# ljanyst/ssd-tensorflow

Measured on AMD Instinct MI355X. Metric: images/sec (fwd+bwd) vgg300 batch32, higher is better.
Workload: dtype f32; 1 GPU; vgg300 training step (forward + multibox loss + backward + momentum update), 32 images/GPU x 1 GPU, synthetic 300x300 BGR 0..255, GPU-encoded labels, Xavier-init weights (BASELINE.json configs[1]); global_batch=32, parallelism=dp1, allreduce=none

## Files before the change

### include/ssdvgg_hip.h

```cpp
#ifndef SSDVGG_HIP_H
#define SSDVGG_HIP_H

#include <stddef.h>

#ifdef __cplusplus
extern "C" {
#endif

typedef struct ssd_net* ssd_handle;

const char* ssd_last_error(void);
const char* ssd_version(void);

int ssd_preset_info(const char* preset, int* image_w, int* image_h, int* num_anchors, int* num_maps);
int ssd_preset_map(const char* preset, int map, int* size, double* scale, int* num_types);

int ssd_anchors(const char* preset, int device, double* out);
int ssd_anchors_abs(const char* preset, int device, int* out);

int ssd_jaccard_overlap(int device, const double* box, const double* boxes, int n, double* iou_out);

int ssd_encode_labels(const char* preset, int num_classes, int device, const double* gt_boxes,
                      const int* gt_cls, const int* gt_offsets, int b, float* vec_out);
int ssd_encode_labels_dev(const char* preset, int num_classes, int device, const double* gt_boxes,
// ... 231 lines not shown

size_t ssd_arena_floats(const char* preset, int num_classes);
int ssd_create(const char* preset, int num_classes, int max_batch, int device, int training,
               unsigned long long seed, float* ext_params_dev, float* ext_grads_dev,
               float* ext_momentum_dev, ssd_handle* out);
#define SSD_DTYPE_F32 0
#define SSD_DTYPE_BF16 1
#define SSD_DTYPE_FP8 2
#define SSD_DTYPE_MXFP8 3
#define SSD_DTYPE_MXFP6 4
int ssd_create_dtype(const char* preset, int num_classes, int max_batch, int device, int training,
                     unsigned long long seed, float* ext_params_dev, float* ext_grads_dev,
                     float* ext_momentum_dev, int dtype, ssd_handle* out);
int ssd_get_dtype(ssd_handle h, int* dtype);
#define SSD_GRAPH_A_TROUS 0
#define SSD_GRAPH_FC 1
size_t ssd_arena_floats_graph(const char* preset, int num_classes, int graph);
int ssd_create_graph(const char* preset, int num_classes, int max_batch, int device, int training,
                     unsigned long long seed, float* ext_params_dev, float* ext_grads_dev,
                     float* ext_momentum_dev, int dtype, int graph, ssd_handle* out);
int ssd_graph(ssd_handle h, int* graph);
int ssd_destroy(ssd_handle h);
int ssd_set_stream(ssd_handle h, void* stream);

int ssd_num_variables(ssd_handle h);
int ssd_variable_info(ssd_handle h, int i, char* name, int name_cap, int* ndim, int shape[4]);
int ssd_load_variable(ssd_handle h, const char* name, const float* data, size_t count);
int ssd_save_variable(ssd_handle h, const char* name, float* data, size_t count);
int ssd_save_gradient(ssd_handle h, const char* name, float* data, size_t count);
int ssd_save_momentum(ssd_handle h, const char* name, float* data, size_t count);
int ssd_load_momentum(ssd_handle h, const char* name, const float* data, size_t count);

int ssd_set_optimizer(ssd_handle h, const float* lr_values, const long long* lr_boundaries,
                      int n_values, float momentum, float weight_decay);
int ssd_get_global_step(ssd_handle h, long long* step);
int ssd_set_global_step(ssd_handle h, long long step);

int ssd_train_step(ssd_handle h, const float* x, const float* y, int b, float* result_out,
                   float losses_out[4]);
int ssd_eval_step(ssd_handle h, const float* x, const float* y, int b, float* result_out,
                  float losses_out[4]);
int ssd_infer(ssd_handle h, const float* x, int b, float* result_out);

int ssd_forward_backward_dev(ssd_handle h, const float* x_dev, const float* y_dev, int b);
int ssd_apply_gradients_dev(ssd_handle h, float grad_scale);
int ssd_forward_dev(ssd_handle h, const float* x_dev, const float* y_dev, int b);
int ssd_backward_begin_dev(ssd_handle h, const float* y_dev, int b);
int ssd_backward_next_dev(ssd_handle h, size_t min_floats, int sync_main, size_t* offset, size_t* count, int* more);
int ssd_backward_ranges(ssd_handle h, size_t min_floats, size_t* offsets, size_t* counts, int cap, int* n_out);
int ssd_set_wgrad_stream(ssd_handle h, void* stream);
int ssd_set_loss_normalizer(ssd_handle h, float batch);
int ssd_null_gradients_dev(ssd_handle h);
enum { SSD_LOSS_MINING = 0, SSD_LOSS_FOCAL = 1 };
typedef struct { int kind; float focal_gamma; float focal_alpha; } ssd_loss_config;
int ssd_set_loss(ssd_handle h, const ssd_loss_config* cfg);
int ssd_get_loss(ssd_handle h, ssd_loss_config* cfg);
enum { SSD_LOC_SMOOTH_L1 = 0, SSD_LOC_GIOU = 1 };
typedef struct { int kind; float weight; } ssd_loc_loss_config;
int ssd_set_loc_loss(ssd_handle h, const ssd_loc_loss_config* cfg);
int ssd_get_loc_loss(ssd_handle h, ssd_loc_loss_config* cfg);

int ssd_grads_to_bf16(int device, const float* grads_dev, void* msg_dev, size_t count, void* stream);
int ssd_grads_from_bf16(int device, const void* msg_dev, float* grads_dev, size_t count, void* stream);
int ssd_train_step_dev(ssd_handle h, const float* x_dev, const float* y_dev, int b);
int ssd_eval_step_dev(ssd_handle h, const float* x_dev, const float* y_dev, int b);
int ssd_infer_dev(ssd_handle h, const float* x_dev, int b);
int ssd_result_dev(ssd_handle h, const float** result_dev);
int ssd_get_losses(ssd_handle h, float losses_out[4]);
int ssd_get_losses_step(ssd_handle h, int steps_back, float losses_out[4]);
int ssd_get_result(ssd_handle h, int b, float* result_out);
int ssd_set_result_dev(ssd_handle h, const float* pred_dev, int b);
int ssd_arenas(ssd_handle h, float** params_dev, float** grads_dev, float** momentum_dev,
               size_t* floats, size_t* filter_floats);
int ssd_detect_last(ssd_handle h, int b, float conf_thr, int cap, int max_out, int out_cap, int nms,
                    int* count, float* conf, int* cls, int* idx, int* box);
int ssd_detect_last_dev(ssd_handle h, int b, float conf_thr, int cap, int max_out, int out_cap, int nms,
                        int** count_dev, float** conf_dev, int** cls_dev, int** idx_dev, int** box_dev);
int ssd_detect_fetch(ssd_handle h, int which, int* count, float* conf, int* cls, int* idx, int* box);
int ssd_detect_last_all_dev(ssd_handle h, int b, float conf_thr, int nms_top_k, int keep_top_k, int out_cap,
                            int** count_dev, float** conf_dev, int** cls_dev, int** idx_dev, int** box_dev);
int ssd_detect_host(ssd_handle h, int which, const int** count, const float** conf, const int** cls, const int** idx,
                    const int** box, int* b, int* out_cap);
int ssd_set_overlap(ssd_handle h, int on);
int ssd_profile_enable(ssd_handle h, int on);
int ssd_profile_report(ssd_handle h, char* buf, size_t cap);
int ssd_activation_shape(ssd_handle h, const char* name, int* height, int* width, int* channels);
int ssd_activation(ssd_handle h, const char* name, int b, float* out, size_t count);

int ssd_op_conv2d_fwd(const float* x, const float* w, const float* bias, float* y, int b, int hi,
                      int wi, int ci, int ho, int wo, int co, int kh, int kw, int stride, int dil,
                      int pad_h, int pad_w, int relu, void* stream);
int ssd_op_conv2d_dgrad(const float* dy, const float* w, float* dx, const float* mask,
                        int accumulate, int b, int hi, int wi, int ci, int ho, int wo, int co,
                        int kh, int kw, int stride, int dil, int pad_h, int pad_w, void* stream);
size_t ssd_op_conv2d_wgrad_ws_floats(int b, int hi, int wi, int ci, int ho, int wo, int co, int kh,
                                     int kw, int stride, int dil, int pad_h, int pad_w);
int ssd_op_conv2d_wgrad(const float* x, const float* dy, float* dw, float* dbias, const float* w,
                        float weight_decay, float* ws, int b, int hi, int wi, int ci, int ho, int wo,
                        int co, int kh, int kw, int stride, int dil, int pad_h, int pad_w,
                        void* stream);
int ssd_op_cast_filter(const float* w, void* w_io_bf16, void* w_oi_bf16, int taps, int ci, int co,
                       void* stream);
int ssd_op_conv2d_fwd_bf16(const void* x, const void* w_oi, const float* bias, void* y, int y_f32,
                           int b, int hi, int wi, int ci, int ho, int wo, int co, int kh, int kw,
                           int stride, int dil, int pad_h, int pad_w, int relu, void* stream);
int ssd_op_conv2d_dgrad_bf16(const void* dy, const void* w_io, void* dx, const void* mask,
                             int accumulate, int b, int hi, int wi, int ci, int ho, int wo, int co,
                             int kh, int kw, int stride, int dil, int pad_h, int pad_w, void* stream);
size_t ssd_op_conv2d_wgrad_bf16_ws_floats(int b, int hi, int wi, int ci, int ho, int wo, int co,
                                          int kh, int kw, int stride, int dil, int pad_h, int pad_w);
int ssd_op_conv2d_wgrad_bf16(const void* x, const void* dy, float* dw, float* dbias, const float* w,
                             float weight_decay, float* ws, int b, int hi, int wi, int ci, int ho,
                             int wo, int co, int kh, int kw, int stride, int dil, int pad_h,
                             int pad_w, void* stream);
int ssd_op_conv2d_fwd_bf16_chain(const void* x, const void* w_oi, const float* bias, void* y, int y_f32,
                                 int b, int hi, int wi, int ci, int ho, int wo, int co, int kh, int kw,
                                 int stride, int dil, int pad_h, int pad_w, int relu, void* stream);
int ssd_op_conv2d_dgrad_bf16_chain(const void* dy, const void* w_io, void* dx, const void* mask,
                                   int accumulate, int b, int hi, int wi, int ci, int ho, int wo, int co,
                                   int kh, int kw, int stride, int dil, int pad_h, int pad_w, void* stream);
int ssd_op_conv2d_wgrad_bf16_direct(const void* x, const void* dy, float* dw, float* dbias, const float* w,
                                    float weight_decay, int b, int hi, int wi, int ci, int ho, int wo, int co,
                                    int kh, int kw, int stride, int dil, int pad_h, int pad_w, void* stream);
typedef struct {
    int hi, wi, ci, ho, wo, co, kh, kw, stride, dil, pad_h, pad_w;
    int dgrad, relu, accum, out_f32;
    const void* src;
    const void* wgt;
    const float* bias;
    const void* mask;
    void* dst;
} ssd_tail_stage;
#define SSD_TAIL_ZERO_BYTES 2560
#define SSD_TAIL_LDS_MAX (160 * 1024)
#define SSD_TAIL_MAX_TASKS 64
#define SSD_TF_RELU 1
#define SSD_TF_ACCUM 2
#define SSD_TF_OUT_F32 4
#define SSD_TF_LOAD_IN 8
#define SSD_TF_LOAD_OUT 16
#define SSD_TF_KTAIL 32
typedef struct {
    int flags;
    int ntask, tiles, ksplit, ngroups, gpt;
    int in_off, in_bytes;
    int out_off, out_bytes;
    int scratch_off, scratch_bytes;
    unsigned tasks[SSD_TAIL_MAX_TASKS][2];
} ssd_tail_plan_stage;
int ssd_op_tail_chain_plan(const ssd_tail_stage* stages, int nstages, ssd_tail_plan_stage* plan_out, int* lds_total_out);
int ssd_op_tail_chain_bf16(const ssd_tail_stage* stages, int nstages, int b, void* stream);
typedef struct {
    int hi, wi, ci, ho, wo, co, kh, kw, stride, dil, pad_h, pad_w;
    const void* x;
    const void* dy;
    float* dw;
    float* dbias;
    const float* w;
} ssd_wgrad_item;
int ssd_op_conv2d_wgrad_group_bf16(const ssd_wgrad_item* items, int n, float weight_decay, int b, void* stream);
int ssd_op_conv2d_first_fwd_bf16(const float* x, const float* w, const float* bias, void* y, int b, int hi,
                                 int wi, int ci, int ho, int wo, int co, int kh, int kw, int stride,
                                 int dil, int pad_h, int pad_w, int relu, void* stream);
size_t ssd_op_conv2d_first_wgrad_bf16_ws_floats(int b, int hi, int wi, int ci, int ho, int wo, int co,
                                                int kh, int kw, int stride, int dil, int pad_h, int pad_w);
int ssd_op_conv2d_first_wgrad_bf16(const float* x, const void* dy, float* dw, float* dbias, const float* w,
// ... 2 lines not shown
                                   int pad_w, void* stream);
int ssd_fp8_calibrate_dev(ssd_handle h, const float* x_dev, int b, int accumulate);
int ssd_fp8_num_scales(ssd_handle h, int* count);
int ssd_fp8_scale_name(ssd_handle h, int i, char* name, int name_cap);
int ssd_fp8_get_scales(ssd_handle h, float* scales, int count);
int ssd_fp8_set_scales(ssd_handle h, const float* scales, int count);
#define SSD_FP8_OUT_BF16 0
#define SSD_FP8_OUT_F32 1
#define SSD_FP8_OUT_E4M3 2
#define SSD_FP8_OUT_BF16_E4M3 3
int ssd_op_quantize_fp8(const void* x, int x_f32, size_t n, float scale, void* y8, void* stream);
int ssd_op_absmax_bf16(const void* x, size_t n, float* out_dev, int accumulate, void* stream);
int ssd_op_quantize_filter_fp8(const float* w, void* w8, float* s_w, int taps, int ci, int co, void* stream);
int ssd_op_conv2d_fwd_fp8(const void* x8, const void* w8, float s_in, const float* s_w, const float* bias, void* y, void* y8,
                          int out_mode, float s_out, int b, int hi, int wi, int ci, int ho, int wo, int co, int kh, int kw,
                          int stride, int dil, int pad_h, int pad_w, int relu, void* stream);
int ssd_op_conv2d_fwd_fp8_bigk(const void* x8, const void* w8, float s_in, const float* s_w, const float* bias, void* y, void* y8,
                               int out_mode, float s_out, int b, int hi, int wi, int ci, int ho, int wo, int co, int kh, int kw,
                               int stride, int dil, int pad_h, int pad_w, int relu, void* stream);
int ssd_op_maxpool_fwd_fp8(const void* x8, void* y8, int b, int hi, int wi, int c, int ho, int wo, int k, int stride,
                           int pad_h, int pad_w, void* stream);
#define SSD_FP8_OUT_MX 4
#define SSD_FP8_OUT_BF16_MX 5
int ssd_op_quantize_mxfp8(const void* x, int x_f32, size_t rows, int c, void* y8, void* yscales, void* stream);
int ssd_op_conv2d_fwd_mxfp8(const void* x8, const void* xscales, const void* w8, const float* s_w, const float* bias, void* y, void* y8,
                            void* yscales, int out_mode, int b, int hi, int wi, int ci, int ho, int wo, int co, int kh, int kw,
                            int stride, int dil, int pad_h, int pad_w, int relu, void* stream);
int ssd_op_conv2d_fwd_mxfp8_bigk(const void* x8, const void* xscales, const void* w8, const float* s_w, const float* bias,
                                 void* y, void* y8, void* yscales, int out_mode,
                                 int b, int hi, int wi, int ci, int ho, int wo, int co, int kh, int kw,
                                 int stride, int dil, int pad_h, int pad_w, int relu, void* stream);
int ssd_op_maxpool_fwd_mxfp8(const void* x8, const void* xscales, void* y8, void* yscales, int b, int hi, int wi, int c, int ho, int wo,
                             int k, int stride, int pad_h, int pad_w, void* stream);
int ssd_op_quantize_mxfp6(const void* x, int x_f32, size_t rows, int c, void* y6, void* yscales, void* stream);
int ssd_op_quantize_filter_mxfp6(const float* w, void* w6, void* wscales, int taps, int ci, int co, void* stream);
int ssd_op_conv2d_fwd_mxfp6(const void* x6, const void* xscales, const void* w6, const void* wscales, const float* bias, void* y, void* y6,
                            void* yscales, int out_mode, int b, int hi, int wi, int ci, int ho, int wo, int co, int kh, int kw,
                            int stride, int dil, int pad_h, int pad_w, int relu, void* stream);
int ssd_op_maxpool_fwd_mxfp6(const void* x6, const void* xscales, void* y6, void* yscales, int b, int hi, int wi, int c, int ho, int wo,
                             int k, int stride, int pad_h, int pad_w, void* stream);
int ssd_op_maxpool_fwd(const float* x, float* y, int b, int hi, int wi, int c, int ho, int wo, int k,
                       int stride, int pad_h, int pad_w, void* stream);
int ssd_op_maxpool_bwd(const float* x, const float* dy, float* dx, int accumulate, int relu_mask,
                       int b, int hi, int wi, int c, int ho, int wo, int k, int stride, int pad_h,
                       int pad_w, void* stream);
int ssd_op_maxpool_fwd_bf16(const void* x, void* y, int b, int hi, int wi, int c, int ho, int wo, int k,
                            int stride, int pad_h, int pad_w, void* stream);
int ssd_op_maxpool_bwd_bf16(const void* x, const void* dy, void* dx, int accumulate, int relu_mask,
                            int b, int hi, int wi, int c, int ho, int wo, int k, int stride, int pad_h,
                            int pad_w, void* stream);
int ssd_op_maxpool_arg_fwd(const void* x, void* y, void* arg, int bf16, int b, int hi, int wi, int c, void* stream);
int ssd_op_maxpool_arg_bwd(const void* x, const void* arg, const void* dy, void* dx, int accumulate, int relu_mask, int bf16,
                           int b, int hi, int wi, int c, void* stream);
int ssd_op_maxpool_rec_fwd(const void* x, void* y, void* rec, int bf16, int b, int hi, int wi, int c, void* stream);
int ssd_op_maxpool_rec_bwd(const void* rec, const void* dy, void* dx, int relu_mask, int bf16, int b, int hi, int wi, int c,
                           void* stream);
int ssd_op_conv2d_fwd_pool(const float* x, const float* w, const float* bias, float* y_pool, void* rec, int b, int hi, int wi,
                           int ci, int ho, int wo, int co, int kh, int kw, int stride, int dil, int pad_h, int pad_w, void* stream);
int ssd_op_conv2d_fwd_pool_bf16(const void* x, const void* w_oi, const float* bias, void* y_pool, void* rec, int b, int hi, int wi,
                                int ci, int ho, int wo, int co, int kh, int kw, int stride, int dil, int pad_h, int pad_w,
                                void* stream);
int ssd_op_conv2d_dgrad_unpool(const float* dy, const float* w, float* dx_unpooled, const void* rec, int uh, int uw, int b, int hi,
                               int wi, int ci, int ho, int wo, int co, int kh, int kw, int stride, int dil, int pad_h, int pad_w,
                               void* stream);
int ssd_op_conv2d_dgrad_unpool_bf16(const void* dy, const void* w_io, void* dx_unpooled, const void* rec, int uh, int uw, int b,
                                    int hi, int wi, int ci, int ho, int wo, int co, int kh, int kw, int stride, int dil, int pad_h,
                                    int pad_w, void* stream);
size_t ssd_op_conv2d_dgrad_first_wgrad_bf16_ws_floats(int b, int h, int w);
int ssd_op_conv2d_dgrad_first_wgrad_bf16(const void* dy, const void* w_io, const void* mask, const float* image, float* dw1, float* dbias1,
                                         const float* w1, float weight_decay, float* ws, int b, int h, int w, void* stream);
size_t ssd_op_conv2d_wino_bits_words(int b, int hi, int wi, int ci, int ho, int wo, int co, int kh, int kw, int stride, int dil,
                                     int pad_h, int pad_w);
size_t ssd_op_conv2d_wino_ws_floats(int b, int hi, int wi, int ci, int ho, int wo, int co, int kh, int kw, int stride, int dil,
                                    int pad_h, int pad_w);
int ssd_op_conv2d_wino_fwd(const float* x, const float* w, const float* bias, float* y, float* y_pool, void* rec, void* relu_bits, float* ws,
                           int flags, int b, int hi, int wi, int ci, int ho, int wo, int co, int kh, int kw, int stride, int dil,
                           int pad_h, int pad_w, int relu, void* stream);
int ssd_op_conv2d_wino_dgrad(const float* dy, const float* w, float* dx, const float* mask, const void* mask_bits, int accumulate,
                             const void* rec, int uh, int uw, float* ws, int flags, int b, int hi, int wi, int ci, int ho, int wo, int co,
                             int kh, int kw, int stride, int dil, int pad_h, int pad_w, void* stream);
int ssd_op_conv2d_wino_wgrad(const float* x, const float* dy, float* dw, float* dbias, const float* w, float weight_decay, float* ws,
                             int flags, int b, int hi, int wi, int ci, int ho, int wo, int co, int kh, int kw, int stride, int dil,
                             int pad_h, int pad_w, void* stream);
int ssd_pool_fusion(ssd_handle h, int* out, int cap, int* count);
int ssd_debug_set_ablate(const char* tokens);

int ssd_op_clock_monitor(unsigned* out_dev, int nsamples, unsigned period_ticks, void* stream);
int ssd_op_l2norm_fwd(const float* x, const float* scale, float* y, int npix, int c, void* stream);
size_t ssd_op_l2norm_bwd_ws_floats(int npix, int c);
int ssd_op_l2norm_bwd(const float* x, const float* scale, const float* dy, float* dx, float* dscale,
                      float* ws, int npix, int c, void* stream);
int ssd_op_l2norm_fwd_bf16(const void* x, const float* scale, void* y, int npix, int c, void* stream);
int ssd_op_l2norm_bwd_bf16(const void* x, const float* scale, const void* dy, void* dx, float* dscale,
                           float* ws, int npix, int c, void* stream);

size_t ssd_op_multibox_loss_ws_bytes(int nmaps, const int* hw, const int* nj, int b_total, size_t* offsets, int* num_anchors);
int ssd_op_multibox_loss(int nmaps, const int* hw, const int* nj, int num_classes, void* const* heads, const float* labels,
                         float* result, void* ws, int b, int b_off, int b_total, float bnorm, const float* filters,
                         size_t nfilters, float weight_decay, void* stream);
int ssd_op_multibox_loss_grad(int nmaps, const int* hw, const int* nj, int num_classes, void* const* grads, int grads_bf16,
                              const float* labels, const float* result, void* ws, int b, int b_off, int b_total, void* stream);
int ssd_op_multibox_loss_ex(int nmaps, const int* hw, const int* nj, int num_classes, void* const* heads, const float* labels,
                            float* result, void* ws, int b, int b_off, int b_total, float bnorm, const float* filters,
                            size_t nfilters, float weight_decay, const ssd_loss_config* cfg, void* stream);
int ssd_op_multibox_loss_grad_ex(int nmaps, const int* hw, const int* nj, int num_classes, void* const* grads, int grads_bf16,
                                 const float* labels, const float* result, void* ws, int b, int b_off, int b_total,
                                 const ssd_loss_config* cfg, void* stream);
int ssd_op_multibox_loss_ex2(int nmaps, const int* hw, const int* nj, int num_classes, void* const* heads, const float* labels,
                             float* result, void* ws, int b, int b_off, int b_total, float bnorm, const float* filters,
                             size_t nfilters, float weight_decay, const ssd_loss_config* cfg, const ssd_loc_loss_config* loc,
                             void* stream);
int ssd_op_multibox_loss_grad_ex2(int nmaps, const int* hw, const int* nj, int num_classes, void* const* grads, int grads_bf16,
                                  const float* labels, const float* result, void* ws, int b, int b_off, int b_total,
                                  const ssd_loss_config* cfg, const ssd_loc_loss_config* loc, void* stream);

#ifdef __cplusplus
}
#endif
#endif
```

### ssd_tensorflow_amd/_lib.py

```python
import ctypes as C
import os

_HERE = os.path.dirname(os.path.abspath(__file__))
LIB_PATH = os.environ.get('SSD_LIB') or os.path.join(_HERE, 'libssdvgg_hip.so')

if not os.path.exists(LIB_PATH):
    raise ImportError(
        f'{LIB_PATH} is missing: build it with `python -c "import __graft_entry__ as g; g.build()"` '
        f'or `make -C {os.path.join(_HERE, "csrc")}` (hipcc, gfx950). There is no CPU fallback.')

try:
    import torch
except ImportError:
    torch = None

lib = C.CDLL(LIB_PATH)

p_f32 = C.POINTER(C.c_float)
p_f64 = C.POINTER(C.c_double)
p_i32 = C.POINTER(C.c_int)
p_i64 = C.POINTER(C.c_longlong)
vp = C.c_void_p
i32 = C.c_int
f32 = C.c_float
# ... 71 lines not shown
    'ssd_annotate_style_destroy': (i32, [vp]),
    'ssd_annotate_ws_bytes': (sz, [i32, i32]),
    'ssd_annotate_batch_dev': (i32, [vp, i32, vp, i32, vp, vp, vp, i32, i32, vp, i32, vp, i32, vp, vp]),
    'ssd_jpeg_info': (i32, [vp, sz, p_i32, p_i32, p_i32, p_i32, p_i32]),
    'ssd_jpeg_coef_bytes': (sz, [vp, sz]),
    'ssd_jpeg_entropy_decode': (i32, [vp, sz, vp, sz, vp, p_i32]),
    'ssd_jpeg_entropy_decode_batch': (i32, [vp, vp, i32, i32, vp, vp, vp, vp]),
    'ssd_jpeg_ws_bytes': (sz, [vp, i32]),
    'ssd_jpeg_decode_batch_dev': (i32, [vp, sz, vp, i32, vp, sz, vp, sz, vp]),
    'ssd_jpeg_scan_segments': (sz, [vp, sz]),
    'ssd_jpeg_scan_plan': (i32, [vp, sz, vp, vp, p_i32]),
    'ssd_jpeg_huffdec_ws_bytes': (sz, [vp, vp, i32]),
    'ssd_jpeg_huffdec_batch_dev': (i32, [vp, sz, vp, vp, i32, vp, sz, vp, vp, sz, i32, vp]),
    'ssd_jpeg_quant_tables': (i32, [i32, vp, vp]),
    'ssd_jpeg_enc_coef_bytes': (sz, [vp, i32, i32]),
    'ssd_jpeg_enc_ws_bytes': (sz, [vp, i32, i32]),
    'ssd_jpeg_encode_batch_dev': (i32, [vp, sz, vp, vp, i32, i32, i32, vp, sz, vp, vp, sz, vp]),
    'ssd_jpeg_file_bound': (sz, [vp]),
    'ssd_jpeg_entropy_encode': (i32, [vp, sz, vp, vp, sz, C.POINTER(sz)]),
    'ssd_jpeg_entropy_encode_batch': (i32, [vp, sz, vp, i32, i32, vp, sz, vp, vp]),
    'ssd_jpeg_file_header': (i32, [vp, vp]),
    'ssd_jpeg_huff_ws_bytes': (sz, [vp, i32]),
    'ssd_jpeg_huff_out_bytes': (sz, [vp, i32]),
    'ssd_jpeg_huffman_batch_dev': (i32, [vp, sz, vp, i32, vp, sz, vp, vp, sz, vp]),
    'ssd_sampler_trials': (i32, [vp, i32, vp, vp, i32, i32, vp, i32, vp, vp]),
    'ssd_create': (i32, [cstr, i32, i32, i32, i32, C.c_ulonglong, vp, vp, vp, C.POINTER(handle)]),
    'ssd_create_dtype': (i32, [cstr, i32, i32, i32, i32, C.c_ulonglong, vp, vp, vp, i32, C.POINTER(handle)]),
    'ssd_get_dtype': (i32, [handle, p_i32]),
    'ssd_arena_floats_graph': (sz, [cstr, i32, i32]),
    'ssd_create_graph': (i32, [cstr, i32, i32, i32, i32, C.c_ulonglong, vp, vp, vp, i32, i32, C.POINTER(handle)]),
    'ssd_graph': (i32, [handle, p_i32]),
    'ssd_destroy': (i32, [handle]),
    'ssd_set_stream': (i32, [handle, vp]),
    'ssd_num_variables': (i32, [handle]),
    'ssd_variable_info': (i32, [handle, i32, C.c_char_p, i32, p_i32, p_i32]),
    'ssd_load_variable': (i32, [handle, cstr, vp, sz]),
    'ssd_save_variable': (i32, [handle, cstr, vp, sz]),
    'ssd_save_gradient': (i32, [handle, cstr, vp, sz]),
    'ssd_save_momentum': (i32, [handle, cstr, vp, sz]),
    'ssd_load_momentum': (i32, [handle, cstr, vp, sz]),
    'ssd_set_optimizer': (i32, [handle, vp, vp, i32, f32, f32]),
    'ssd_get_global_step': (i32, [handle, p_i64]),
    'ssd_set_global_step': (i32, [handle, C.c_longlong]),
    'ssd_train_step': (i32, [handle, vp, vp, i32, vp, vp]),
    'ssd_eval_step': (i32, [handle, vp, vp, i32, vp, vp]),
    'ssd_infer': (i32, [handle, vp, i32, vp]),
    'ssd_forward_backward_dev': (i32, [handle, vp, vp, i32]),
    'ssd_apply_gradients_dev': (i32, [handle, f32]),
    'ssd_forward_dev': (i32, [handle, vp, vp, i32]),
    'ssd_backward_begin_dev': (i32, [handle, vp, i32]),
    'ssd_backward_next_dev': (i32, [handle, sz, i32, C.POINTER(sz), C.POINTER(sz), p_i32]),
    'ssd_backward_ranges': (i32, [handle, sz, C.POINTER(sz), C.POINTER(sz), i32, p_i32]),
    'ssd_set_wgrad_stream': (i32, [handle, vp]),
    'ssd_set_loss_normalizer': (i32, [handle, f32]),
    'ssd_null_gradients_dev': (i32, [handle]),
    'ssd_set_loss': (i32, [handle, vp]),
    'ssd_get_loss': (i32, [handle, vp]),
    'ssd_set_loc_loss': (i32, [handle, vp]),
    'ssd_get_loc_loss': (i32, [handle, vp]),
    'ssd_train_step_dev': (i32, [handle, vp, vp, i32]),
    'ssd_eval_step_dev': (i32, [handle, vp, vp, i32]),
    'ssd_infer_dev': (i32, [handle, vp, i32]),
    'ssd_result_dev': (i32, [handle, C.POINTER(vp)]),
    'ssd_get_result': (i32, [handle, i32, vp]),
    'ssd_get_losses': (i32, [handle, vp]),
    'ssd_get_losses_step': (i32, [handle, i32, vp]),
    'ssd_set_result_dev': (i32, [handle, vp, i32]),
    'ssd_arenas': (i32, [handle, C.POINTER(vp), C.POINTER(vp), C.POINTER(vp), C.POINTER(sz), C.POINTER(sz)]),
    'ssd_detect_last': (i32, [handle, i32, f32, i32, i32, i32, i32, vp, vp, vp, vp, vp]),
    'ssd_detect_last_dev': (i32, [handle, i32, f32, i32, i32, i32, i32, C.POINTER(vp), C.POINTER(vp), C.POINTER(vp), C.POINTER(vp), C.POINTER(vp)]),
    'ssd_detect_last_all_dev': (i32, [handle, i32, f32, i32, i32, i32, C.POINTER(vp), C.POINTER(vp), C.POINTER(vp), C.POINTER(vp), C.POINTER(vp)]),
    'ssd_detect_fetch': (i32, [handle, i32, vp, vp, vp, vp, vp]),
    'ssd_detect_host': (i32, [handle, i32, C.POINTER(vp), C.POINTER(vp), C.POINTER(vp), C.POINTER(vp), C.POINTER(vp), p_i32, p_i32]),
    'ssd_nms_boxes': (i32, [i32, i32, vp, vp, vp, C.c_double, vp, p_i32]),
    'ssd_merge_tiles_limits': (i32, [p_i32, p_i32, p_i32]),
    'ssd_merge_tiles_ws_bytes': (sz, [i32, i32]),
    'ssd_merge_tiles_dev': (i32, [vp, i32, i32, i32, vp, vp, vp, vp, vp, i32, i32, i32, vp, vp, vp, vp, vp, vp, vp, vp]),
    'ssd_merge_tiles': (i32, [i32, vp, i32, i32, i32, vp, vp, vp, vp, vp, i32, i32, i32, vp, vp, vp, vp, vp, vp]),
    'ssd_detout_tiles_ws_bytes': (sz, [cstr, i32, i32, i32, i32]),
    'ssd_detout_tiles_add_dev': (i32, [cstr, i32, vp, vp, vp, i32, i32, i32, f32, i32, i32, vp, sz, vp]),
    'ssd_detout_tiles_merge_dev': (i32, [i32, vp, i32, i32, i32, i32, i32, vp, vp, vp, vp, vp, vp, vp, sz, vp]),
    'ssd_detout_tiles': (i32, [cstr, i32, i32, vp, vp, i32, i32, f32, i32, i32, i32, i32, vp, vp, vp, vp, vp, vp]),
    'ssd_set_overlap': (i32, [handle, i32]),
    'ssd_profile_enable': (i32, [handle, i32]),
    'ssd_profile_report': (i32, [handle, C.c_char_p, sz]),
    'ssd_activation_shape': (i32, [handle, cstr, p_i32, p_i32, p_i32]),
    'ssd_activation': (i32, [handle, cstr, i32, vp, sz]),
    'ssd_op_conv2d_fwd': (i32, [vp, vp, vp, vp] + [i32] * 14 + [vp]),
    'ssd_op_conv2d_dgrad': (i32, [vp, vp, vp, vp, i32] + [i32] * 13 + [vp]),
    'ssd_op_conv2d_wgrad_ws_floats': (sz, [i32] * 13),
    'ssd_op_conv2d_wgrad': (i32, [vp, vp, vp, vp, vp, f32, vp] + [i32] * 13 + [vp]),
    'ssd_op_conv2d_wino_ws_floats': (sz, [i32] * 13),
    'ssd_op_conv2d_wino_bits_words': (sz, [i32] * 13),
    'ssd_op_conv2d_wino_fwd': (i32, [vp, vp, vp, vp, vp, vp, vp, vp, i32] + [i32] * 14 + [vp]),
    'ssd_op_conv2d_wino_dgrad': (i32, [vp, vp, vp, vp, vp, i32, vp, i32, i32, vp, i32] + [i32] * 13 + [vp]),
    'ssd_op_conv2d_wino_wgrad': (i32, [vp, vp, vp, vp, vp, f32, vp, i32] + [i32] * 13 + [vp]),
    'ssd_op_cast_filter': (i32, [vp, vp, vp, i32, i32, i32, vp]),
    'ssd_op_conv2d_fwd_bf16': (i32, [vp, vp, vp, vp, i32] + [i32] * 14 + [vp]),
    'ssd_op_conv2d_dgrad_bf16': (i32, [vp, vp, vp, vp, i32] + [i32] * 13 + [vp]),
    'ssd_op_conv2d_fwd_bf16_chain': (i32, [vp, vp, vp, vp, i32] + [i32] * 14 + [vp]),
    'ssd_op_conv2d_dgrad_bf16_chain': (i32, [vp, vp, vp, vp, i32] + [i32] * 13 + [vp]),
    'ssd_op_conv2d_wgrad_bf16_direct': (i32, [vp, vp, vp, vp, vp, f32] + [i32] * 13 + [vp]),
    'ssd_op_tail_chain_plan': (i32, [C.POINTER(TailStage), i32, C.POINTER(TailPlanStage), p_i32]),
    'ssd_op_tail_chain_bf16': (i32, [C.POINTER(TailStage), i32, i32, vp]),
    'ssd_op_conv2d_wgrad_group_bf16': (i32, [C.POINTER(WgradItem), i32, f32, i32, vp]),
    'ssd_op_conv2d_wgrad_bf16_ws_floats': (sz, [i32] * 13),
    'ssd_op_conv2d_wgrad_bf16': (i32, [vp, vp, vp, vp, vp, f32, vp] + [i32] * 13 + [vp]),
    'ssd_op_conv2d_first_fwd_bf16': (i32, [vp, vp, vp, vp] + [i32] * 14 + [vp]),
    'ssd_op_conv2d_first_wgrad_bf16_ws_floats': (sz, [i32] * 13),
    'ssd_op_conv2d_first_wgrad_bf16': (i32, [vp, vp, vp, vp, vp, f32, vp] + [i32] * 13 + [vp]),
    'ssd_op_maxpool_rec_fwd': (i32, [vp, vp, vp, i32, i32, i32, i32, i32, vp]),
    'ssd_op_maxpool_rec_bwd': (i32, [vp, vp, vp, i32, i32, i32, i32, i32, i32, vp]),
    'ssd_op_conv2d_fwd_pool': (i32, [vp, vp, vp, vp, vp] + [i32] * 13 + [vp]),
    'ssd_op_conv2d_fwd_pool_bf16': (i32, [vp, vp, vp, vp, vp] + [i32] * 13 + [vp]),
    'ssd_op_conv2d_dgrad_unpool': (i32, [vp, vp, vp, vp, i32, i32] + [i32] * 13 + [vp]),
    'ssd_op_conv2d_dgrad_unpool_bf16': (i32, [vp, vp, vp, vp, i32, i32] + [i32] * 13 + [vp]),
    'ssd_op_conv2d_dgrad_first_wgrad_bf16_ws_floats': (sz, [i32, i32, i32]),
    'ssd_op_conv2d_dgrad_first_wgrad_bf16': (i32, [vp, vp, vp, vp, vp, vp, vp, f32, vp, i32, i32, i32, vp]),
    'ssd_pool_fusion': (i32, [handle, p_i32, i32, p_i32]),
    'ssd_debug_set_ablate': (i32, [cstr]),
    'ssd_fp8_calibrate_dev': (i32, [handle, vp, i32, i32]),
    'ssd_fp8_num_scales': (i32, [handle, p_i32]),
    'ssd_fp8_scale_name': (i32, [handle, i32, C.c_char_p, i32]),
    'ssd_fp8_get_scales': (i32, [handle, vp, i32]),
    'ssd_fp8_set_scales': (i32, [handle, vp, i32]),
    'ssd_op_quantize_fp8': (i32, [vp, i32, sz, f32, vp, vp]),
    'ssd_op_absmax_bf16': (i32, [vp, sz, vp, i32, vp]),
    'ssd_op_quantize_filter_fp8': (i32, [vp, vp, vp, i32, i32, i32, vp]),
    'ssd_op_conv2d_fwd_fp8': (i32, [vp, vp, f32, vp, vp, vp, vp, i32, f32] + [i32] * 14 + [vp]),
    'ssd_op_conv2d_fwd_fp8_bigk': (i32, [vp, vp, f32, vp, vp, vp, vp, i32, f32] + [i32] * 14 + [vp]),
    'ssd_op_maxpool_fwd_fp8': (i32, [vp, vp] + [i32] * 10 + [vp]),
    'ssd_op_quantize_mxfp8': (i32, [vp, i32, sz, i32, vp, vp, vp]),
    'ssd_op_conv2d_fwd_mxfp8': (i32, [vp, vp, vp, vp, vp, vp, vp, vp, i32] + [i32] * 14 + [vp]),
    'ssd_op_conv2d_fwd_mxfp8_bigk': (i32, [vp, vp, vp, vp, vp, vp, vp, vp, i32] + [i32] * 14 + [vp]),
    'ssd_op_maxpool_fwd_mxfp8': (i32, [vp, vp, vp, vp] + [i32] * 10 + [vp]),
    'ssd_op_quantize_mxfp6': (i32, [vp, i32, sz, i32, vp, vp, vp]),
    'ssd_op_quantize_filter_mxfp6': (i32, [vp, vp, vp, i32, i32, i32, vp]),
    'ssd_op_conv2d_fwd_mxfp6': (i32, [vp, vp, vp, vp, vp, vp, vp, vp, i32] + [i32] * 14 + [vp]),
    'ssd_op_maxpool_fwd_mxfp6': (i32, [vp, vp, vp, vp] + [i32] * 10 + [vp]),
    'ssd_op_maxpool_fwd': (i32, [vp, vp] + [i32] * 10 + [vp]),
    'ssd_op_maxpool_bwd': (i32, [vp, vp, vp, i32, i32] + [i32] * 10 + [vp]),
    'ssd_op_maxpool_fwd_bf16': (i32, [vp, vp] + [i32] * 10 + [vp]),
    'ssd_op_maxpool_bwd_bf16': (i32, [vp, vp, vp, i32, i32] + [i32] * 10 + [vp]),
    'ssd_op_maxpool_arg_fwd': (i32, [vp, vp, vp, i32, i32, i32, i32, i32, vp]),
    'ssd_op_maxpool_arg_bwd': (i32, [vp, vp, vp, vp, i32, i32, i32, i32, i32, i32, i32, vp]),
    'ssd_op_clock_monitor': (i32, [vp, i32, C.c_uint, vp]),
    'ssd_grads_to_bf16': (i32, [i32, vp, vp, sz, vp]),
    'ssd_grads_from_bf16': (i32, [i32, vp, vp, sz, vp]),
    'ssd_op_l2norm_fwd': (i32, [vp, vp, vp, i32, i32, vp]),
    'ssd_op_l2norm_bwd_ws_floats': (sz, [i32, i32]),
    'ssd_op_l2norm_bwd': (i32, [vp, vp, vp, vp, vp, vp, i32, i32, vp]),
    'ssd_op_l2norm_fwd_bf16': (i32, [vp, vp, vp, i32, i32, vp]),
    'ssd_op_l2norm_bwd_bf16': (i32, [vp, vp, vp, vp, vp, vp, i32, i32, vp]),
    'ssd_op_multibox_loss_ws_bytes': (sz, [i32, p_i32, p_i32, i32, C.POINTER(sz), p_i32]),
    'ssd_op_multibox_loss': (i32, [i32, p_i32, p_i32, i32, C.POINTER(vp), vp, vp, vp, i32, i32, i32, f32, vp, sz, f32, vp]),
    'ssd_op_multibox_loss_grad': (i32, [i32, p_i32, p_i32, i32, C.POINTER(vp), i32, vp, vp, vp, i32, i32, i32, vp]),
    'ssd_op_multibox_loss_ex': (i32, [i32, p_i32, p_i32, i32, C.POINTER(vp), vp, vp, vp, i32, i32, i32, f32, vp, sz, f32, vp, vp]),
    'ssd_op_multibox_loss_grad_ex': (i32, [i32, p_i32, p_i32, i32, C.POINTER(vp), i32, vp, vp, vp, i32, i32, i32, vp, vp]),
    'ssd_op_multibox_loss_ex2': (i32, [i32, p_i32, p_i32, i32, C.POINTER(vp), vp, vp, vp, i32, i32, i32, f32, vp, sz, f32, vp, vp, vp]),
    'ssd_op_multibox_loss_grad_ex2': (i32, [i32, p_i32, p_i32, i32, C.POINTER(vp), i32, vp, vp, vp, i32, i32, i32, vp, vp, vp]),
}

for _name, (_res, _args) in SIGNATURES.items():
    _fn = getattr(lib, _name)
    _fn.restype = _res
    _fn.argtypes = _args


_device = 0


def set_device(device):
    global _device
    _device = int(device)


def device():
    return _device

# ... 17 lines not shown
```

### ssd_tensorflow_amd/csrc/api.hip

```cpp
#include "../../include/ssdvgg_hip.h"
#include "net.h"
#include "augment.h"
#include "annotate.h"
#include "jpeg.h"
#include "jpeg_enc.h"
#include "jpeg_huff.h"
#include "jpeg_huffdec.h"
#include "metrics.h"
#include <vector>
#include <map>
#include <memory>
#include <mutex>
#include <algorithm>

namespace ssd {
static thread_local std::string g_err;
void set_error(const char* fmt, ...) {
    char buf[1024];
    va_list ap;
    va_start(ap, fmt);
    vsnprintf(buf, sizeof buf, fmt, ap);
    va_end(ap);
    g_err = buf;
}
// ... 1283 lines not shown
    n.forward(n.x_stage(), b, true, n.y_stage());
    n.backward_apply(b, n.y_stage(), 1.f);
    if (result_out) n.copy_result(result_out, b);
    if (losses_out) n.get_losses(losses_out);
    HIP_OK(hipStreamSynchronize(n.stream()));
    API_END
}
int ssd_eval_step(ssd_handle h, const float* x, const float* y, int b, float* result_out, float losses_out[4]) {
    API_BEGIN_NET(h)
    n.upload_xy(x, y, b);
    n.forward(n.x_stage(), b, true, n.y_stage());
    if (result_out) n.copy_result(result_out, b);
    if (losses_out) n.get_losses(losses_out);
    HIP_OK(hipStreamSynchronize(n.stream()));
    API_END
}
int ssd_infer(ssd_handle h, const float* x, int b, float* result_out) {
    API_BEGIN_NET(h)
    n.upload_xy(x, nullptr, b);
    n.forward(n.x_stage(), b, false, nullptr);
    if (result_out) n.copy_result(result_out, b);
    HIP_OK(hipStreamSynchronize(n.stream()));
    API_END
}

int ssd_detect_last(ssd_handle h, int b, float conf_thr, int cap, int max_out, int out_cap, int nms, int* count, float* conf,
                    int* cls, int* idx, int* box) {
    API_BEGIN_NET(h)
    n.detect_last(b, conf_thr, cap, max_out, out_cap, nms != 0, count, conf, cls, idx, box);
    API_END
}

int ssd_detect_last_dev(ssd_handle h, int b, float conf_thr, int cap, int max_out, int out_cap, int nms, int** count_dev,
                        float** conf_dev, int** cls_dev, int** idx_dev, int** box_dev) {
    API_BEGIN_NET(h)
    DetectOut d{};
    n.detect_last_dev(b, conf_thr, cap, max_out, out_cap, nms != 0, &d);
    if (count_dev) *count_dev = d.count;
    if (conf_dev) *conf_dev = d.conf;
    if (cls_dev) *cls_dev = d.cls;
    if (idx_dev) *idx_dev = d.idx;
    if (box_dev) *box_dev = d.box;
    API_END
}

int ssd_detect_last_all_dev(ssd_handle h, int b, float conf_thr, int nms_top_k, int keep_top_k, int out_cap, int** count_dev,
                            float** conf_dev, int** cls_dev, int** idx_dev, int** box_dev) {
    API_BEGIN_NET(h)
    DetectOut d{};
    n.detect_last_all_dev(b, conf_thr, nms_top_k, keep_top_k, out_cap, &d);
    if (count_dev) *count_dev = d.count;
    if (conf_dev) *conf_dev = d.conf;
    if (cls_dev) *cls_dev = d.cls;
    if (idx_dev) *idx_dev = d.idx;
    if (box_dev) *box_dev = d.box;
    API_END
}

int ssd_detect_fetch(ssd_handle h, int which, int* count, float* conf, int* cls, int* idx, int* box) {
    API_BEGIN_NET(h)
    n.detect_fetch(which, count, conf, cls, idx, box);
    API_END
}

int ssd_detect_host(ssd_handle h, int which, const int** count, const float** conf, const int** cls, const int** idx,
                    const int** box, int* b, int* out_cap) {
    API_BEGIN_NET(h)
    DetectOut d;
    n.detect_host(which, &d, b, out_cap);
    if (count) *count = d.count;
    if (conf) *conf = d.conf;
    if (cls) *cls = d.cls;
    if (idx) *idx = d.idx;
    if (box) *box = d.box;
    API_END
}

int ssd_set_overlap(ssd_handle h, int on) {
    API_BEGIN_NET(h)
    n.set_overlap(on != 0);
    API_END
}

int ssd_profile_enable(ssd_handle h, int on) {
    API_BEGIN_NET(h)
    n.profiler().on = on != 0;
    n.profiler().detailed = on == 2;
    n.profiler().reset();
    API_END
}

int ssd_profile_report(ssd_handle h, char* buf, size_t cap) {
    API_BEGIN_NET(h)
    HIP_OK(hipStreamSynchronize(n.stream()));
    struct Agg { long long cnt = 0; double ms = 0, fl = 0, by = 0; };
    std::map<std::string, Agg> agg;
    for (const auto& r : n.profiler().recs) {
        float ms = 0.f;
        HIP_OK(hipEventElapsedTime(&ms, r.e0, r.e1));
        Agg& a = agg[r.kernel];
        a.cnt++; a.ms += ms; a.fl += r.flops; a.by += r.bytes;
    }
    std::string out;
    char line[384];
    for (const auto& kv : agg) {
        snprintf(line, sizeof line, "%s\t%lld\t%.6f\t%.6e\t%.6e\n", kv.first.c_str(), kv.second.cnt, kv.second.ms, kv.second.fl,
                 kv.second.by);
        out += line;
    }
    SSD_REQUIRE(buf && cap > out.size(), "report needs %zu bytes", out.size() + 1);
    memcpy(buf, out.c_str(), out.size() + 1);
    n.profiler().reset();
    API_END
}

int ssd_activation_shape(ssd_handle h, const char* name, int* height, int* width, int* channels) {
    API_BEGIN_NET(h)
    n.activation_shape(name, height, width, channels);
    API_END
}

int ssd_activation(ssd_handle h, const char* name, int b, float* out, size_t count) {
    API_BEGIN_NET(h)
    n.activation(name, b, out, count);
    API_END
}

static ConvDesc mk(int b, int hi, int wi, int ci, int ho, int wo, int co, int kh, int kw, int stride, int dil, int pad_h,
                   int pad_w) {
    ConvDesc d;
    d.B = b; d.Hi = hi; d.Wi = wi; d.Ci = ci; d.Ho = ho; d.Wo = wo; d.Co = co;
    d.KH = kh; d.KW = kw; d.stride = stride; d.dil = dil; d.pad_h = pad_h; d.pad_w = pad_w;
    return d;
}

int ssd_op_conv2d_fwd(const float* x, const float* w, const float* bias, float* y, int b, int hi, int wi, int ci, int ho,
                      int wo, int co, int kh, int kw, int stride, int dil, int pad_h, int pad_w, int relu, void* stream) {
    API_BEGIN
    conv_fwd(mk(b, hi, wi, ci, ho, wo, co, kh, kw, stride, dil, pad_h, pad_w), x, w, bias, y, relu != 0, (hipStream_t)stream);
    API_END
}
int ssd_op_conv2d_dgrad(const float* dy, const float* w, float* dx, const float* mask, int accumulate, int b, int hi, int wi,
                        int ci, int ho, int wo, int co, int kh, int kw, int stride, int dil, int pad_h, int pad_w,
                        void* stream) {
    API_BEGIN
    conv_dgrad(mk(b, hi, wi, ci, ho, wo, co, kh, kw, stride, dil, pad_h, pad_w), dy, w, dx, mask, accumulate != 0,
               (hipStream_t)stream);
    API_END
}
int ssd_op_cast_filter(const float* w, void* w_io_bf16, void* w_oi_bf16, int taps, int ci, int co, void* stream) {
    API_BEGIN
    FilterCastPlan plan;
    plan.add(0, taps, ci, co);
    cast_filters(plan, w, (bf16_t*)w_io_bf16, (bf16_t*)w_oi_bf16, (hipStream_t)stream);
    API_END
}
int ssd_op_conv2d_fwd_bf16(const void* x, const void* w_oi, const float* bias, void* y, int y_f32, int b, int hi, int wi, int ci,
                           int ho, int wo, int co, int kh, int kw, int stride, int dil, int pad_h, int pad_w, int relu,
                           void* stream) {
    API_BEGIN
    conv_fwd_bf16(mk(b, hi, wi, ci, ho, wo, co, kh, kw, stride, dil, pad_h, pad_w), (const bf16_t*)x, (const bf16_t*)w_oi, bias, y,
                  y_f32 != 0, relu != 0, (hipStream_t)stream);
    API_END
}
int ssd_op_conv2d_dgrad_bf16(const void* dy, const void* w_io, void* dx, const void* mask, int accumulate, int b, int hi, int wi,
                             int ci, int ho, int wo, int co, int kh, int kw, int stride, int dil, int pad_h, int pad_w,
// ... 133 lines not shown
    API_BEGIN
    conv_first_fwd_bf16(mk(b, hi, wi, ci, ho, wo, co, kh, kw, stride, dil, pad_h, pad_w), x, w, bias, (bf16_t*)y, relu != 0,
                        (hipStream_t)stream);
    API_END
}
size_t ssd_op_conv2d_first_wgrad_bf16_ws_floats(int b, int hi, int wi, int ci, int ho, int wo, int co, int kh, int kw, int stride,
                                                int dil, int pad_h, int pad_w) {
    return conv_first_wgrad_bf16_ws_floats(mk(b, hi, wi, ci, ho, wo, co, kh, kw, stride, dil, pad_h, pad_w));
}
int ssd_op_conv2d_first_wgrad_bf16(const float* x, const void* dy, float* dw, float* dbias, const float* w, float weight_decay,
                                   float* ws, int b, int hi, int wi, int ci, int ho, int wo, int co, int kh, int kw, int stride,
                                   int dil, int pad_h, int pad_w, void* stream) {
    API_BEGIN
    conv_first_wgrad_bf16(mk(b, hi, wi, ci, ho, wo, co, kh, kw, stride, dil, pad_h, pad_w), x, (const bf16_t*)dy, dw, dbias, w,
                          weight_decay, ws, (hipStream_t)stream);
    API_END
}
namespace {
struct WinoWs {
    float *U, *Uf, *V, *Mx, *Yt, *Ya, *slabs;
    size_t total;
    WinoWs(const ConvDesc& d, float* ws) {
        const size_t cop = wino_kpad(d.Co), u = (size_t)36 * d.Ci * cop, t = (size_t)36 * wino_tiles(d);
        U = ws; Uf = U + u; V = Uf + u; Mx = V + t * d.Ci; Yt = Mx + t * std::max((size_t)d.Ci, cop); Ya = Yt + t * cop; slabs = Ya + t * cop;
        total = (size_t)(slabs - ws) + wino_wgrad_ws_floats(d);
    }
};
}
size_t ssd_op_conv2d_wino_ws_floats(int b, int hi, int wi, int ci, int ho, int wo, int co, int kh, int kw, int stride, int dil,
                                    int pad_h, int pad_w) {
    const ConvDesc d = mk(b, hi, wi, ci, ho, wo, co, kh, kw, stride, dil, pad_h, pad_w);
    return wino_applicable(d) ? WinoWs(d, nullptr).total : 0;
}
size_t ssd_op_conv2d_wino_bits_words(int b, int hi, int wi, int ci, int ho, int wo, int co, int kh, int kw, int stride, int dil,
                                     int pad_h, int pad_w) {
    const ConvDesc d = mk(b, hi, wi, ci, ho, wo, co, kh, kw, stride, dil, pad_h, pad_w);
    return wino_applicable(d) ? (size_t)wino_tiles(d) * (d.Ci / 4) : 0;
}
int ssd_op_conv2d_wino_fwd(const float* x, const float* w, const float* bias, float* y, float* y_pool, void* rec, void* relu_bits, float* ws,
                           int flags, int b, int hi, int wi, int ci, int ho, int wo, int co, int kh, int kw, int stride, int dil,
                           int pad_h, int pad_w, int relu, void* stream) {
    API_BEGIN
    const ConvDesc d = mk(b, hi, wi, ci, ho, wo, co, kh, kw, stride, dil, pad_h, pad_w);
    SSD_REQUIRE(wino_applicable(d), "winograd: 3x3 / stride 1 / SAME layers (any dilation), Ci in multiples of 32, Co of 4");
    const WinoWs k(d, ws);
    if (!(flags & 1)) {
        HIP_OK(hipMemsetAsync(k.Uf, 0, (size_t)36 * d.Ci * wino_kpad(d.Co) * sizeof(float), (hipStream_t)stream));
        wino_filter(d, w, k.U, k.Uf, (hipStream_t)stream);
    }
    wino_fwd(d, x, k.U, bias, y, relu != 0, k.V, (size_t)wino_tiles(d) * d.Ci, k.Mx, y_pool, rec, (hipStream_t)stream, relu_bits,
             (flags & 4) != 0, (flags & 8) != 0);
    API_END
}
int ssd_op_conv2d_wino_dgrad(const float* dy, const float* w, float* dx, const float* mask, const void* mask_bits, int accumulate,
                             const void* rec, int uh, int uw, float* ws, int flags, int b, int hi, int wi, int ci, int ho, int wo, int co,
                             int kh, int kw, int stride, int dil, int pad_h, int pad_w, void* stream) {
    API_BEGIN
    const ConvDesc d = mk(b, hi, wi, ci, ho, wo, co, kh, kw, stride, dil, pad_h, pad_w);
    SSD_REQUIRE(wino_applicable(d), "winograd: 3x3 / stride 1 / SAME layers (any dilation), Ci in multiples of 32, Co of 4");
    const WinoWs k(d, ws);
    if (!(flags & 1)) {
        HIP_OK(hipMemsetAsync(k.Uf, 0, (size_t)36 * d.Ci * wino_kpad(d.Co) * sizeof(float), (hipStream_t)stream));
        wino_filter(d, w, k.U, k.Uf, (hipStream_t)stream);
    }
    wino_bwd_transform(d, dy, k.Yt, nullptr, (hipStream_t)stream, (flags & 8) != 0);
    wino_dgrad(d, k.Yt, k.Uf, dx, mask, accumulate != 0, k.Mx, rec, uh, uw, (hipStream_t)stream, mask_bits, (flags & 4) != 0);
    API_END
}
int ssd_op_conv2d_wino_wgrad(const float* x, const float* dy, float* dw, float* dbias, const float* w, float weight_decay, float* ws,
                             int flags, int b, int hi, int wi, int ci, int ho, int wo, int co, int kh, int kw, int stride, int dil,
                             int pad_h, int pad_w, void* stream) {
    API_BEGIN
    const ConvDesc d = mk(b, hi, wi, ci, ho, wo, co, kh, kw, stride, dil, pad_h, pad_w);
    SSD_REQUIRE(wino_applicable(d), "winograd: 3x3 / stride 1 / SAME layers (any dilation), Ci in multiples of 32, Co of 4");
    const WinoWs k(d, ws);
    const size_t vps = (size_t)wino_tiles(d) * d.Ci;
    if (!(flags & 2)) {
        ConvDesc dx = d;
        dx.Co = d.Ci; dx.Ho = d.Hi; dx.Wo = d.Wi;
        wino_bwd_transform(dx, x, k.V, nullptr, (hipStream_t)stream, (flags & 8) != 0);
    }
    wino_bwd_transform(d, dy, nullptr, k.Ya, (hipStream_t)stream, (flags & 8) != 0);
    wino_wgrad(d, k.V, vps, k.Ya, dw, dbias, w, weight_decay, k.slabs, (hipStream_t)stream, (flags & 8) != 0);
    API_END
}
size_t ssd_op_conv2d_wgrad_ws_floats(int b, int hi, int wi, int ci, int ho, int wo, int co, int kh, int kw, int stride,
                                     int dil, int pad_h, int pad_w) {
    return conv_wgrad_ws_floats(mk(b, hi, wi, ci, ho, wo, co, kh, kw, stride, dil, pad_h, pad_w));
}
int ssd_op_conv2d_wgrad(const float* x, const float* dy, float* dw, float* dbias, const float* w, float weight_decay,
                        float* ws, int b, int hi, int wi, int ci, int ho, int wo, int co, int kh, int kw, int stride, int dil,
                        int pad_h, int pad_w, void* stream) {
    API_BEGIN
    conv_wgrad(mk(b, hi, wi, ci, ho, wo, co, kh, kw, stride, dil, pad_h, pad_w), x, dy, dw, dbias, w, weight_decay, ws,
               (hipStream_t)stream);
    API_END
}
int ssd_op_quantize_fp8(const void* x, int x_f32, size_t n, float scale, void* y8, void* stream) {
    API_BEGIN
    quantize_fp8(x, x_f32 != 0, n, scale, (unsigned char*)y8, (hipStream_t)stream);
    API_END
}
int ssd_op_absmax_bf16(const void* x, size_t n, float* out_dev, int accumulate, void* stream) {
    API_BEGIN
    absmax_bf16((const bf16_t*)x, n, out_dev, accumulate != 0, (hipStream_t)stream);
    API_END
}
int ssd_op_quantize_filter_fp8(const float* w, void* w8, float* s_w, int taps, int ci, int co, void* stream) {
    API_BEGIN
    SSD_REQUIRE(w && w8 && s_w && taps >= 1 && ci >= 1 && co >= 1, "quantize_filter_fp8: null argument or empty filter");
    FilterQuantPlan plan;
    plan.add(0, 0, 0, taps, ci, co);
    quantize_filters_fp8(plan, w, (unsigned char*)w8, s_w, (hipStream_t)stream);
    API_END
}
int ssd_op_conv2d_fwd_fp8(const void* x8, const void* w8, float s_in, const float* s_w, const float* bias, void* y, void* y8,
                          int out_mode, float s_out, int b, int hi, int wi, int ci, int ho, int wo, int co, int kh, int kw, int stride,
                          int dil, int pad_h, int pad_w, int relu, void* stream) {
    API_BEGIN
    conv_fwd_fp8(mk(b, hi, wi, ci, ho, wo, co, kh, kw, stride, dil, pad_h, pad_w), (const unsigned char*)x8, (const unsigned char*)w8, s_in,
                 s_w, bias, y, (unsigned char*)y8, out_mode, s_out, relu != 0, (hipStream_t)stream);
    API_END
}
int ssd_op_conv2d_fwd_fp8_bigk(const void* x8, const void* w8, float s_in, const float* s_w, const float* bias, void* y, void* y8,
                               int out_mode, float s_out, int b, int hi, int wi, int ci, int ho, int wo, int co, int kh, int kw, int stride,
                               int dil, int pad_h, int pad_w, int relu, void* stream) {
    API_BEGIN
    conv_bigk_fwd_fp8(mk(b, hi, wi, ci, ho, wo, co, kh, kw, stride, dil, pad_h, pad_w), (const unsigned char*)x8, (const unsigned char*)w8,
                      s_in, s_w, bias, y, (unsigned char*)y8, out_mode, s_out, relu != 0, (hipStream_t)stream);
    API_END
}
int ssd_op_maxpool_fwd_fp8(const void* x8, void* y8, int b, int hi, int wi, int c, int ho, int wo, int k, int stride, int pad_h,
                           int pad_w, void* stream) {
    API_BEGIN
    PoolDesc d{b, hi, wi, c, ho, wo, k, stride, pad_h, pad_w};
    maxpool_fwd_fp8(d, (const unsigned char*)x8, (unsigned char*)y8, (hipStream_t)stream);
    API_END
}
int ssd_op_quantize_mxfp8(const void* x, int x_f32, size_t rows, int c, void* y8, void* yscales, void* stream) {
    API_BEGIN
    quantize_mxfp8(x, x_f32 != 0, rows, c, (unsigned char*)y8, (unsigned char*)yscales, (hipStream_t)stream);
    API_END
}
int ssd_op_conv2d_fwd_mxfp8(const void* x8, const void* xscales, const void* w8, const float* s_w, const float* bias, void* y, void* y8,
                            void* yscales, int out_mode, int b, int hi, int wi, int ci, int ho, int wo, int co, int kh, int kw, int stride,
                            int dil, int pad_h, int pad_w, int relu, void* stream) {
    API_BEGIN
    conv_fwd_mxfp8(mk(b, hi, wi, ci, ho, wo, co, kh, kw, stride, dil, pad_h, pad_w), (const unsigned char*)x8, (const unsigned char*)xscales,
                   (const unsigned char*)w8, s_w, bias, y, (unsigned char*)y8, (unsigned char*)yscales, out_mode, relu != 0, (hipStream_t)stream);
    API_END
}
int ssd_op_conv2d_fwd_mxfp8_bigk(const void* x8, const void* xscales, const void* w8, const float* s_w, const float* bias, void* y, void* y8,
                                 void* yscales, int out_mode, int b, int hi, int wi, int ci, int ho, int wo, int co, int kh, int kw, int stride,
                                 int dil, int pad_h, int pad_w, int relu, void* stream) {
    API_BEGIN
    conv_bigk_fwd_mxfp8(mk(b, hi, wi, ci, ho, wo, co, kh, kw, stride, dil, pad_h, pad_w), (const unsigned char*)x8, (const unsigned char*)xscales,
                        (const unsigned char*)w8, s_w, bias, y, (unsigned char*)y8, (unsigned char*)yscales, out_mode, relu != 0, (hipStream_t)stream);
    API_END
}
int ssd_op_maxpool_fwd_mxfp8(const void* x8, const void* xscales, void* y8, void* yscales, int b, int hi, int wi, int c, int ho, int wo, int k,
                             int stride, int pad_h, int pad_w, void* stream) {
    API_BEGIN
    PoolDesc d{b, hi, wi, c, ho, wo, k, stride, pad_h, pad_w};
    maxpool_fwd_mxfp8(d, (const unsigned char*)x8, (const unsigned char*)xscales, (unsigned char*)y8, (unsigned char*)yscales, (hipStream_t)stream);
    API_END
}
// ... 334 lines not shown
```

### ssd_tensorflow_amd/csrc/conv.h

```cpp
#pragma once
#include <vector>
#include "common.h"

namespace ssd {

struct ConvDesc {
    int B, Hi, Wi, Ci;
    int Ho, Wo, Co;
    int KH, KW, stride, dil;
    int pad_h, pad_w;
};

void conv_fwd(const ConvDesc& d, const float* x, const float* w, const float* bias,
              float* y, bool relu, hipStream_t s);

void conv_dgrad(const ConvDesc& d, const float* dy, const float* w, float* dx,
                const float* mask, bool accumulate, hipStream_t s);

size_t conv_wgrad_ws_floats(const ConvDesc& d);
void conv_wgrad(const ConvDesc& d, const float* x, const float* dy, float* dw, float* dbias,
                const float* w, float weight_decay, float* ws, hipStream_t s);

bool conv_fwd_pool_supported(const ConvDesc& d);
void conv_fwd_pool(const ConvDesc& d, const float* x, const float* w, const float* bias, float* y_pool, void* rec, hipStream_t s);
bool conv_dgrad_unpool_supported(const ConvDesc& d);
void conv_dgrad_unpool(const ConvDesc& d, const float* dy, const float* w, float* dx_unpooled, const void* rec, int UH, int UW,
                       hipStream_t s);

bool conv_first_fwd_f32_applicable(const ConvDesc& d);
void conv_first_fwd_f32(const ConvDesc& d, const float* x, const float* w, const float* bias, float* y, bool relu, hipStream_t s);
bool conv_first_wgrad_f32_applicable(const ConvDesc& d);
size_t conv_first_wgrad_f32_ws_floats(const ConvDesc& d);
void conv_first_wgrad_f32(const ConvDesc& d, const float* x, const float* dy, float* dw, float* dbias, const float* w,
                          float weight_decay, float* ws, hipStream_t s);

bool wino_applicable(const ConvDesc& d);
int wino_tiles(const ConvDesc& d);
int wino_kpad(int c);
void wino_filter(const ConvDesc& d, const float* w, float* U, float* Uflip, hipStream_t s);
struct WinoFilterPlan {
    static constexpr int MAX = 24;
    struct Item {
        const float* w;
        float *U, *Uf;
        int Ci, Co, Cop, blk0;
    } it[MAX];
    int n = 0, blocks = 0;
    double elems = 0;
    void add(const float* w, float* U, float* Uf, int Ci, int Co);
};
void wino_filter_plan(const WinoFilterPlan& plan, bool forward, bool flipped, hipStream_t s);
size_t wino_fwd_ws_floats(const ConvDesc& d);
void wino_fwd(const ConvDesc& d, const float* x, const float* U, const float* bias, float* y, bool relu, float* V, size_t v_ps,
              float* Mws, float* y_pool, void* pool_rec, hipStream_t s, void* relu_bits = nullptr, bool two_launch = false,
              bool ref_geom = false);
void wino_bwd_transform(const ConvDesc& d, const float* dy, float* Yt, float* Ya, hipStream_t s, bool ref_geom = false);
size_t wino_dgrad_ws_floats(const ConvDesc& d);
void wino_dgrad(const ConvDesc& d, const float* Yt, const float* Uflip, float* dx, const float* mask, bool accumulate, float* Xws,
                const void* unpool_rec, int UH, int UW, hipStream_t s, const void* mask_bits = nullptr, bool two_launch = false);
size_t wino_wgrad_ws_floats(const ConvDesc& d);
void wino_wgrad(const ConvDesc& d, const float* V, size_t v_ps, const float* Ya, float* dw, float* dbias, const float* w,
                float weight_decay, float* ws, hipStream_t s, bool ref_geom = false);

bool conv_bigk(const ConvDesc& d);
double conv_bigk_useful_flops(const ConvDesc& d);
void conv_bigk_fwd(const ConvDesc& d, const float* x, const float* w, const float* bias, float* y, bool relu, hipStream_t s);
void conv_bigk_dgrad(const ConvDesc& d, const float* dy, const float* w, float* dx, const float* mask, bool accumulate, hipStream_t s);
void conv_bigk_wgrad(const ConvDesc& d, const float* x, const float* dy, float* dw, float* dbias, const float* w, float weight_decay,
                     hipStream_t s);

struct bf16_t;

void conv_fwd_smallc_bf16out(const ConvDesc& d, const float* x, const float* w, const float* bias, bf16_t* y, bool relu,
                             hipStream_t s);
void conv_wgrad_smallc_bf16dy(const ConvDesc& d, const float* x, const bf16_t* dy, float* dw, float* dbias, const float* w,
                              float weight_decay, float* ws, hipStream_t s);

void conv_first_fwd_bf16(const ConvDesc& d, const float* x, const float* w, const float* bias, bf16_t* y, bool relu, hipStream_t s);
size_t conv_first_wgrad_bf16_ws_floats(const ConvDesc& d);
void conv_first_wgrad_bf16(const ConvDesc& d, const float* x, const bf16_t* dy, float* dw, float* dbias, const float* w,
                           float weight_decay, float* ws, hipStream_t s);

void conv_bigk_fwd_bf16(const ConvDesc& d, const bf16_t* x, const bf16_t* w_oi, const float* bias, void* y, bool y_f32, bool relu,
                        hipStream_t s);
void conv_bigk_dgrad_bf16(const ConvDesc& d, const bf16_t* dy, const bf16_t* w_io, bf16_t* dx, const bf16_t* mask, bool accumulate,
                          hipStream_t s);
void conv_bigk_wgrad_bf16(const ConvDesc& d, const bf16_t* x, const bf16_t* dy, float* dw, float* dbias, const float* w,
                          float weight_decay, hipStream_t s);

struct FilterCastPlan {
    static constexpr int MAX_LAYERS = 48;
    struct Layer {
        size_t off;
        int taps, ci, co;
    } L[MAX_LAYERS];
    int n = 0;
    void add(size_t off, int taps, int ci, int co);
};
void cast_filters(const FilterCastPlan& plan, const float* w, bf16_t* io, bf16_t* oi, hipStream_t s);

extern thread_local int g_conv_lanes;
void conv_fwd_bf16(const ConvDesc& d, const bf16_t* x, const bf16_t* w_oi, const float* bias, void* y, bool y_f32, bool relu,
                   hipStream_t s);
void conv_dgrad_bf16(const ConvDesc& d, const bf16_t* dy, const bf16_t* w_io, bf16_t* dx, const bf16_t* mask, bool accumulate,
                     hipStream_t s);
bool conv_fwd_pool_bf16_supported(const ConvDesc& d);
void conv_fwd_pool_bf16(const ConvDesc& d, const bf16_t* x, const bf16_t* w_oi, const float* bias, bf16_t* y_pool, void* rec, hipStream_t s);
bool conv_dgrad_unpool_bf16_supported(const ConvDesc& d);
void conv_dgrad_unpool_bf16(const ConvDesc& d, const bf16_t* dy, const bf16_t* w_io, bf16_t* dx_unpooled, const void* rec, int UH, int UW,
                            hipStream_t s);
bool conv_dgrad_first_wgrad_bf16_applicable(const ConvDesc& d, const ConvDesc& d1);
size_t conv_dgrad_first_wgrad_bf16_ws_floats(const ConvDesc& d1);
void conv_dgrad_first_wgrad_bf16(const ConvDesc& d, const bf16_t* dy, const bf16_t* w_io, const bf16_t* mask, const ConvDesc& d1,
                                 const float* image, float* dw1, float* dbias1, const float* w1, float weight_decay, float* ws,
                                 hipStream_t s);
size_t conv_wgrad_bf16_ws_floats(const ConvDesc& d);
void conv_wgrad_bf16(const ConvDesc& d, const bf16_t* x, const bf16_t* dy, float* dw, float* dbias, const float* w,
                     float weight_decay, float* ws, hipStream_t s);

struct TailStage {
    ConvDesc d;
    bool dgrad;
    const void* src;
    const void* wgt_packed;
    const float* bias;
    const void* mask;
    void* dst;
    bool relu, accum, out_f32;
};
int tail_chain_max_stages();
bool tail_chain_stage_supported(const ConvDesc& d);
size_t tail_chain_packed_elems(const ConvDesc& d, bool dgrad);
struct TailPackItem {
    ConvDesc d;
    bool dgrad;
    const void* mirror;
    void* packed;
};
void tail_chain_pack_filters(const TailPackItem* items, int n, hipStream_t s);
// ... 72 lines not shown
```

### ssd_tensorflow_amd/csrc/net.h

```cpp
#pragma once
#include "common.h"
#include "conv.h"
#include "ops.h"
#include "boxes.h"
#include "bf16.h"
#include "quant_layout.h"
#include <string>
#include <vector>
#include <map>

namespace ssd {

struct Tensor {
    std::string name;
    int H = 0, W = 0, C = 0;
    bool relu_out = false;
    int consumers = 0;
    int done = 0;
    int gstream = 0;
    long gseq = 0;
    hipEvent_t gev = nullptr;
    bool gev_set = false;
    bool data_f32 = true;
    bool grad_f32 = true;
// ... 42 lines not shown
    size_t off, rows, width, pitch;
    size_t count() const { return rows * width; }
};

struct DetectSlot {
    char* dev = nullptr;
    char* host = nullptr;
    size_t bytes = 0, used = 0;
    int b = 0, out_cap = 0;
    hipEvent_t ready = nullptr;
};

class Net {
public:
    Net(const char* preset, int num_classes, int max_batch, int device, bool training, unsigned long long seed,
        float* ext_params, float* ext_grads, float* ext_momentum, int dtype = 0, int graph = 0);
    ~Net();

    static size_t arena_floats(const char* preset, int num_classes, int graph = 0);

    void set_stream(hipStream_t s) { stream_ = s; }
    hipStream_t stream() const { return stream_; }

    void forward(const float* x, int b, bool train_mode, const float* y);
    void backward(int b, const float* y);
    void backward_begin(int b, const float* y);
    bool backward_step(size_t min_floats, size_t* off, size_t* count, bool sync_main);
    std::vector<std::pair<size_t, size_t>> backward_ranges(size_t min_floats) const;
    void set_wgrad_stream(hipStream_t s);
    void apply_gradients(float grad_scale);
    void backward_apply(int b, const float* y, float grad_scale);
    void set_loss_normalizer(float bnorm) { loss_bnorm_ = bnorm; }
    void set_loss(int kind, float gamma, float alpha) { loss_kind_ = kind; focal_gamma_ = gamma; focal_alpha_ = alpha; }
    void get_loss(int* kind, float* gamma, float* alpha) const { *kind = loss_kind_; *gamma = focal_gamma_; *alpha = focal_alpha_; }
    void set_loc_loss(int kind, float weight) { loc_.kind = kind; loc_.weight = weight; }
    void get_loc_loss(int* kind, float* weight) const { *kind = loc_.kind; *weight = loc_.weight; }
    void null_gradients_step();
    void set_optimizer(const float* lr_values, const long long* bounds, int n, float momentum, float wd);

    void upload_xy(const float* x, const float* y, int b);
    const float* x_stage() const { return x_stage_; }
    const float* y_stage() const { return y_stage_; }

    void get_losses(float out[4]);
    void get_losses_step(int steps_back, float out[4]);
    void copy_result(float* out, int b);
    void set_result(const float* pred_dev, int b);

    const std::vector<Variable>& variables() const { return vars_; }
    void load_variable(const char* name, const float* host, size_t count, int which);
    void save_variable(const char* name, float* host, size_t count, int which);
    void activation(const char* name, int b, float* out, size_t count);
    void activation_shape(const char* name, int* H, int* W, int* C) const;
    void pool_fusion(int* out, int cap, int* count) const;

    void detect_last(int b, float thr, int cap, int max_out, int out_cap, bool nms, int* count, float* conf, int* cls, int* idx, int* box);
    const DetectSlot& detect_last_dev(int b, float thr, int cap, int max_out, int out_cap, bool nms, DetectOut* dev_out);
    const DetectSlot& detect_last_all_dev(int b, float thr, int nms_top_k, int keep_top_k, int out_cap, DetectOut* dev_out);
    void detect_fetch(int which, int* count, float* conf, int* cls, int* idx, int* box);
    void detect_host(int which, DetectOut* host, int* b, int* out_cap);

    const Preset& preset() const { return *preset_; }
    int num_classes() const { return C_; }
    int nvars() const { return C_ + 5; }
    int max_batch() const { return Bmax_; }
    bool training() const { return training_; }
    int dtype() const { return quant_ == Quant::fp8 ? 2 : quant_ == Quant::mxfp8 ? 3 : quant_ == Quant::mxfp6 ? 4 : bf16_ ? 1 : 0; }
    void fp8_calibrate(const float* x_dev, int b, bool accumulate);
    int fp8_num_scales() const;
    const char* fp8_scale_name(int i) const;
    void fp8_get_scales(float* out, int n) const;
    void fp8_set_scales(const float* v, int n);
    int graph() const { return fc_ ? 1 : 0; }
    int device() const { return device_; }
    float* params() { return params_; }
    float* grads() { return grads_; }
    float* momentum() { return mom_; }
    size_t nparams() const { return nparams_; }
    size_t nfilters() const { return nfilters_; }
    float* result() { return result_; }
    long long global_step = 0;
    Profiler& profiler() { return prof_; }
    void set_overlap(bool on) { overlap_ = on; }

private:
    int add_tensor(const std::string& name, int H, int W, int C, bool relu_out);
    void build_graph();
    void alloc();
    void init_weights(unsigned long long seed);
    ConvDesc conv_desc(const Op& op, int b) const;
    float current_lr() const;
    const Variable& find_var(const char* name) const;

    const Preset* preset_;
    int C_, Bmax_, device_;
    bool training_;
    bool bf16_ = false;
    bool fc_ = false;
    Quant quant_ = Quant::none;
    unsigned char* wsc6_ = nullptr;
    QView q_at(const Tensor& t, int b0) const;
    bool fp8_calibrated_ = false, fp8_as_bf16_ = false;
    unsigned char* w8_ = nullptr;
    float *sw8_ = nullptr, *absmax8_ = nullptr;
    FilterQuantPlan quant_plan_;
    std::vector<int> fp8_scaled_;
    void plan_fp8();
    void fp8_share_pool_scales();
    void require_fp8() const;
    bf16_t *wq_io_ = nullptr, *wq_oi_ = nullptr;
    FilterCastPlan cast_plan_;
    hipStream_t stream_ = nullptr;
    hipStream_t wstream_ = nullptr;
    hipEvent_t ev_dy_ = nullptr, ev_w_ = nullptr;
    hipStream_t hstream_ = nullptr;
    hipEvent_t ev_h_ = nullptr, ev_cast_ = nullptr, ev_fmap_[MAX_MAPS] = {};
    hipStream_t s2_ = nullptr;
    hipEvent_t ev2_h_ = nullptr, ev_l2_ = nullptr, ev_join_ = nullptr, ev2_fmap_[MAX_MAPS] = {};
    int tail_first_ = 0;
    std::vector<int> fwd_order_, bwd_order_;
    struct BwProgress {
        const Net* net = nullptr;
        std::vector<char> done;
        bool chain_done = false;
        int pos = 0;
        size_t hi = 0, lo = 0;
        void begin(const Net* n);
        int next(size_t min_floats);
        bool finished() const;
        size_t retire(int op_index);
        void retire_chain();
        std::pair<size_t, size_t> end_stage();
    private:
        size_t final_lo() const;
    } bw_;
    long bw_issued_[2] = {0, 0}, bw_seen_[2][2] = {{0, 0}, {0, 0}};
    hipEvent_t ev_m2s_ = nullptr;
    bool bw_first_on_main_ = false;
    bool fuse_first_wgrad_ = false;
    bool bw_first_fused_ = false;
    int fused_first_out_ = -1;
    void launch_wgrad(int op_index, int b, hipStream_t ws);
    void launch_dgrad(const Op& op, const ConvDesc& d, const Op* up, Tensor& dst, bool mask, int cls, hipStream_t ds);
    int chain_first_ = -1;
    std::vector<char> in_chain_;
    bf16_t* wq_tail_ = nullptr;
    std::vector<long long> tail_fwd_off_, tail_bwd_off_;
    void pack_tail_filters(hipStream_t s);
    bool chain_fwd_ = false, chain_bwd_ = false;
    void plan_tail_chain();
    void plan_winograd();
    long long fwd_serial_ = 0;
    WinoFilterPlan wino_plan_, wino_plan_first_, wino_plan_flip_;
    bool wino_flip_pending_ = false;
    bool wino_any_f_ = false, wino_any_d_ = false;
    float *wino_m_[3] = {nullptr, nullptr, nullptr}, *wino_vs_[3] = {nullptr, nullptr, nullptr}, *wino_yt_ = nullptr, *wino_xw_ = nullptr, *wino_ya_ = nullptr, *wino_slab_ = nullptr;
    hipEvent_t ev_wino_ = nullptr, ev_wino_first_ = nullptr, ev_wino_flip_ = nullptr;
    struct Lane {
        hipStream_t s, h;
        hipEvent_t* ev_fmap;
        hipEvent_t ev_h;
        int b0, nb;
        bool heads_on_side, cast_pending;
        int wino_pending;
        bool fmap_carried[MAX_MAPS];
    };
    struct FwdPass {
        Lane lane[2];
        int nl, nl_cur;
        bool heads_full;
        int small_heads;
        int b;
        bool train_mode, run8, side;
    };
    struct LossSlotGuard;
    struct ConvRun;
    void forward_filters(FwdPass& p, LossSlotGuard& guard);
    void forward_conv(FwdPass& p, int li, int op_index);
    bool conv_stream(FwdPass& p, int li, const Op& op, ConvRun& r);
    void conv_wino_scratch(const FwdPass& p, int li, int op_index, const ConvDesc& d, ConvRun& r);
    void launch_conv_fwd(const FwdPass& p, const Op& op, const ConvDesc& d, const ConvRun& r);
    void forward_pool(FwdPass& p, int li, int op_index);
    void forward_l2norm(FwdPass& p, int li, int op_index);
    void forward_loss(FwdPass& p, const float* y, LossSlotGuard& guard);
    void launch_tail_forward(int b0, int nb, hipStream_t s);
    void launch_tail_backward(int b, bool* side_used);
    void build_orders();
    void plan_pool_fusion();
    int bw_class(const Op& op, int op_index) const;
    void bw_sync(int x, int y);
    void bw_need(int x, const Tensor& t);
    void bw_wrote(int x, Tensor& t, bool carried = false);
    bool overlap_ = true;

    std::vector<Tensor> tensors_;
    std::vector<Op> ops_;
    std::vector<Variable> vars_;
    int input_t_ = -1;
    std::vector<int> head_t_;
    HeadLayout heads_{};

    size_t nparams_ = 0, nfilters_ = 0, scale_off_ = 0;
    float *params_ = nullptr, *grads_ = nullptr, *mom_ = nullptr;

    float* result_ = nullptr;
    float *x_stage_ = nullptr, *y_stage_ = nullptr;
    float* wgrad_ws_ = nullptr;
    float* l2_ws_ = nullptr;
    void* pool_ws_ = nullptr;
    int pool_arg_op_ = -1;
    void* loss_ws_ = nullptr;
    LossWork lw_{};
    static constexpr int LOSS_RING = 4;
    float* losses_host_ = nullptr;
    float* losses_dev_ = nullptr;
    hipEvent_t ev_loss_[LOSS_RING] = {};
    long long loss_seq_ = -1;
    float* begin_loss_slot();
    double* anchors_dev_ = nullptr;
    int* anchors_abs_dev_ = nullptr;
    void* detect_ws_ = nullptr;
    void* detout_ws_ = nullptr;
    size_t detout_ws_bytes_ = 0;
    DetectSlot& detect_slot_next(int b, int out_cap);
    DetectSlot det_slot_[2];
    int det_cur_ = 0;
    void detect_slot_carve(const DetectSlot& sl, DetectOut& d, char* base) const;

    std::vector<float> lr_values_{0.001f};
    std::vector<long long> lr_bounds_;
    float momentum_ = 0.9f, wd_ = 0.0005f;
    float loss_bnorm_ = 0.f;
    int loss_kind_ = 0;
    int bw_loss_kind_ = 0;
    float focal_gamma_ = 2.f, focal_alpha_ = 0.25f, bw_gamma_ = 2.f, bw_alpha_ = 0.25f;
    LocLoss loc_{}, bw_loc_{};
    Profiler prof_;
    int bw_b_ = 0;
    HipOwner hip_;
    TailTables tail_tables_{hip_, {}};
// ... 4 lines not shown
```

### ssd_tensorflow_amd/csrc/net.hip

```cpp
#include "net.h"
#include <cmath>
#include <algorithm>
#include <cstdlib>
#include <atomic>
#include <mutex>

namespace ssd {

static bool first_layer_kernel(const ConvDesc& d) { return d.Ci * d.KH * d.KW <= 32 && d.Co == 64; }

int Net::add_tensor(const std::string& name, int H, int W, int C, bool relu_out) {
    Tensor t;
    t.name = name; t.H = H; t.W = W; t.C = C; t.relu_out = relu_out;
    tensors_.push_back(t);
    return (int)tensors_.size() - 1;
}

enum PadMode { PAD_SAME, PAD_VALID, PAD_BR1_VALID };

void Net::build_graph() {
    const Preset& p = *preset_;
    const int nv = C_ + 5;
    input_t_ = add_tensor("image_input", p.image_h, p.image_w, 3, false);
    int cur = input_t_;
// ... 389 lines not shown
        t.wgt_packed = wq_tail_ + tail_fwd_off_[oi];
        t.bias = params_ + op.b_off;
        t.dst = static_cast<char*>(out.data) + (size_t)b0 * out.per_image() * (out.data_f32 ? 4 : 2);
        t.relu = op.relu; t.accum = false; t.out_f32 = out.data_f32;
        st.push_back(t);
    }
    prof_.layer = "tail";
    tail_chain_bf16(st.data(), (int)st.size(), nb, "tail_fwd_bf16", s, tail_tables_);
}

void Net::launch_tail_backward(int b, bool* side_used) {
    const bool side = hstream_ && overlap_;
    const int cls = side ? 1 : 0;
    hipStream_t ds = cls == 1 ? hstream_ : stream_;
    std::vector<TailStage> st;
    std::vector<Tensor*> written;
    Tensor* first_out = &tensors_[ops_[chain_first_].out];
    for (const int oi : bwd_order_) {
        if (!in_chain_[oi] || oi == chain_first_) continue;
        const Op& op = ops_[oi];
        Tensor& in = tensors_[op.in];
        const Tensor& out = tensors_[op.out];
        bw_need(cls, out);
        const bool last = in.done + 1 == in.consumers;
        TailStage t{};
        t.d = conv_desc(op, 1);
        t.dgrad = true;
        t.src = out.grad;
        t.wgt_packed = wq_tail_ + tail_bwd_off_[oi];
        t.mask = (last && in.relu_out) ? in.data : nullptr;
        t.dst = in.grad;
        t.accum = in.done > 0;
        st.push_back(t);
        in.done++;
        if (std::find(written.begin(), written.end(), &in) == written.end()) written.push_back(&in);
    }
    prof_.layer = "tail";
    const bool carry = first_out->gev != nullptr;
    g_stop_event = carry ? first_out->gev : nullptr;
    {
        struct Disarm { ~Disarm() { g_stop_event = nullptr; } } disarm;
        tail_chain_bf16(st.data(), (int)st.size(), b, "tail_dgrad_bf16", ds, tail_tables_);
    }
    for (Tensor* t : written) {
        t->gstream = cls;
        t->gseq = ++bw_issued_[cls];
        t->gev_set = false;
    }
    if (carry) first_out->gev_set = true;
    const bool wside = wstream_ && overlap_;
    hipStream_t ws = wside ? wstream_ : stream_;
    if (wside || cls == 1) {
        if (carry) {
            HIP_OK(hipStreamWaitEvent(ws, first_out->gev, 0));
        } else {
            HIP_OK(hipEventRecord(ev_dy_, ds));
            HIP_OK(hipStreamWaitEvent(ws, ev_dy_, 0));
        }
        if (!wside) bw_seen_[0][1] = bw_issued_[1];
    }
    std::vector<WgradGroupItem> items;
    for (int oi = 0; oi < (int)ops_.size(); ++oi) {
        if (!in_chain_[oi]) continue;
        const Op& op = ops_[oi];
        const Tensor& in = tensors_[op.in];
        const Tensor& out = tensors_[op.out];
        WgradGroupItem it{};
        it.d = conv_desc(op, b);
        if (oi == chain_first_) continue;
        it.x = in.h(); it.dy = out.gh();
        it.dw = grads_ + op.w_off; it.dbias = grads_ + op.b_off; it.w = params_ + op.w_off;
        items.push_back(it);
    }
    conv_wgrad_group_bf16(items.data(), (int)items.size(), wd_, ws);
    bw_.retire_chain();
    if (wside) *side_used = true;
}

void Net::plan_winograd() {
    if (bf16_) return;
    const int mode = env_i("SSD_WINOGRAD", 15), min_cc = env_i("SSD_WINO_MIN_CC", 4096), head_min_hw = env_i("SSD_WINO_HEAD_MIN_HW", 16);
    if (!(mode & 7)) return;
    size_t m_max = 0, v_max = 0, yt_max = 0, xw_max = 0, slab_max = 0;
    for (Op& op : ops_) {
        if (op.kind != OP_CONV) continue;
        const ConvDesc d = conv_desc(op, Bmax_);
        if (!wino_applicable(d) || d.Ci * d.Co < min_cc) continue;
        if (d.Ci > 1024) continue;
        if (op.head >= 0 && (d.Ho < head_min_hw || !(mode & 8))) continue;
        op.wino_f = (mode & 1) != 0;
        op.wino_d = (mode & 2) != 0 && training_ && op.in != input_t_;
        op.wino_w = (mode & 4) != 0 && training_ && op.wino_f;
        if (!(op.wino_f || op.wino_d)) continue;
        const size_t u = (size_t)36 * d.Ci * d.Co, uf = (size_t)36 * d.Ci * wino_kpad(d.Co), t = (size_t)36 * wino_tiles(d);
        if (op.wino_f) {
            op.wino_U = (float*)hip_.mem(u * sizeof(float));
            if (training_) op.wino_V = (float*)hip_.mem(t * d.Ci * sizeof(float));
            else v_max = std::max(v_max, t * d.Ci);
            m_max = std::max(m_max, t * d.Co);
        }
        if (op.wino_f && op.wino_d) op.wino_bits = hip_.mem((size_t)wino_tiles(d) * (d.Ci / 4) * 8);
        if (op.wino_d) {
            op.wino_Uf = (float*)hip_.mem(uf * sizeof(float));
            HIP_OK(hipMemset(op.wino_Uf, 0, uf * sizeof(float)));
            yt_max = std::max(yt_max, t * wino_kpad(d.Co));
            xw_max = std::max(xw_max, t * d.Ci);
        }
        if (op.wino_w) {
            yt_max = std::max(yt_max, t * wino_kpad(d.Co));
            for (int b = 1; b <= Bmax_; ++b) slab_max = std::max(slab_max, wino_wgrad_ws_floats(conv_desc(op, b)));
        }
        (wino_plan_first_.n == 0 && op.wino_f ? wino_plan_first_ : wino_plan_).add(params_ + op.w_off, op.wino_U, nullptr, d.Ci, d.Co);
        if (op.wino_Uf) wino_plan_flip_.add(params_ + op.w_off, nullptr, op.wino_Uf, d.Ci, d.Co);
        wino_any_f_ |= op.wino_f;
        wino_any_d_ |= op.wino_d;
    }
    if (wino_plan_.n + wino_plan_first_.n + wino_plan_flip_.n == 0) return;
    ev_wino_ = hip_.event();
    ev_wino_first_ = hip_.event();
    ev_wino_flip_ = hip_.event();
    if (m_max) for (int l = 0; l < 3; ++l) wino_m_[l] = (float*)hip_.mem(m_max * sizeof(float));
    if (v_max) for (int l = 0; l < 3; ++l) wino_vs_[l] = (float*)hip_.mem(v_max * sizeof(float));
    if (training_) {
        wino_yt_ = (float*)hip_.mem(yt_max * sizeof(float));
        wino_xw_ = (float*)hip_.mem(xw_max * sizeof(float));
        wino_ya_ = (float*)hip_.mem(yt_max * sizeof(float));
        wino_slab_ = (float*)hip_.mem(slab_max * sizeof(float));
    }
}

void Net::plan_fp8() {
    size_t nsw = 0;
    for (Tensor& t : tensors_) t.wants16 = false;
    std::vector<int> producer(tensors_.size(), -1);
    for (int i = 0; i < (int)ops_.size(); ++i) {
        Op& op = ops_[i];
        producer[op.out] = i;
        if (op.kind != OP_CONV) continue;
        const ConvDesc d = conv_desc(op, Bmax_);
        const bool kernel8 = !conv_bigk(d) ? conv_fwd_fp8_supported(d, nullptr) && conv_fwd_fp8_worthwhile(d) && (quant_ != Quant::mxfp6 || conv_fwd_mxfp6_supported(d, nullptr))
                             : quant_ == Quant::mxfp6 ? false
                             : quant_ == Quant::mxfp8 ? conv_bigk_fwd_mxfp8_supported(d, FP8_OUT_BF16_MX, nullptr) && conv_bigk_fwd_mxfp8_worthwhile(d)
                                                      : conv_bigk_fwd_fp8_supported(d, nullptr) && conv_bigk_fwd_fp8_worthwhile(d);
        op.fp8 = op.head < 0 && i < tail_first_ && !tensors_[op.in].data_f32 && kernel8;
    }
    auto need8 = [&](Tensor& t) {
        if (!t.data8) t.data8 = static_cast<unsigned char*>(hip_.mem(t.per_image() * Bmax_));
        if (quant_block_scales(quant_) && !t.scale8)
            t.scale8 = static_cast<unsigned char*>(hip_.mem(quant_scale_bytes(quant_, t.per_image()) * Bmax_ + 8));
    };
    for (int i = (int)ops_.size() - 1; i >= 0; --i) {
        Op& op = ops_[i];
        Tensor& in = tensors_[op.in];
        Tensor& out = tensors_[op.out];
        if (op.kind == OP_POOL) {
            const int prod = producer[op.in];
            op.fp8 = out.data8 != nullptr && prod >= 0 && ops_[prod].kind == OP_CONV && ops_[prod].fp8;
            if (op.fp8) {
                need8(in);
                if (out.wants16) in.wants16 = true;
            } else {
                in.wants16 = true;
            }
        } else if (op.kind == OP_CONV && op.fp8) {
            need8(in);
        } else {
            in.wants16 = true;
        }
    }
    for (int t : head_t_) tensors_[t].wants16 = true;
    size_t nw6 = 0;
    for (Op& op : ops_) {
        if (op.kind == OP_CONV && op.fp8 && quant_ == Quant::mxfp6) {
            const Tensor& in = tensors_[op.in];
            const Tensor& out = tensors_[op.out];
            const size_t n = (size_t)op.KH * op.KW * out.C * in.C;
            op.sw_off = nsw;
            op.w8_off = nw6;
            quant_plan_.add(op.w_off, nw6, nsw, op.KH * op.KW, in.C, out.C);
            nw6 += (quant_code_bytes(quant_, n) + 15) / 16 * 16;
            nsw += (quant_scale_bytes(quant_, n) + 15) / 16 * 16;
        } else if (op.kind == OP_CONV && op.fp8) {
            const Tensor& in = tensors_[op.in];
            const Tensor& out = tensors_[op.out];
            op.sw_off = nsw;
            op.w8_off = op.w_off;
            quant_plan_.add(op.w_off, op.w8_off, nsw, op.KH * op.KW, in.C, out.C);
            nsw += out.C;
        }
        Tensor& out = tensors_[op.out];
        if (!out.data8) continue;
        if (!op.fp8) out.wants16 = true;
        if (!(op.kind == OP_POOL && op.fp8) && quant_tensor_scale(quant_)) fp8_scaled_.push_back(op.out);
    }
    SSD_REQUIRE(quant_plan_.n > 0, "no layer of this graph is eligible for fp8");
    if (quant_ == Quant::mxfp6) {
        w8_ = static_cast<unsigned char*>(hip_.mem(nw6));
        wsc6_ = static_cast<unsigned char*>(hip_.mem(nsw + 8));
        return;
    }
    w8_ = static_cast<unsigned char*>(hip_.mem(nfilters_));
    sw8_ = static_cast<float*>(hip_.mem(nsw * sizeof(float)));
    if (quant_tensor_scale(quant_)) absmax8_ = static_cast<float*>(hip_.mem(fp8_scaled_.size() * sizeof(float)));
}

QView Net::q_at(const Tensor& t, int b0) const {
    return QView{t.data8 ? t.data8 + (size_t)b0 * quant_code_bytes(quant_, t.per_image()) : nullptr,
                 t.scale8 ? t.scale8 + (size_t)b0 * quant_scale_bytes(quant_, t.per_image()) : nullptr, t.scale};
}

// ... 144 lines not shown
                }
                op.ws_off = ws_total;
                ws_total += (ws + 63) / 64 * 64;
            }
        wgrad_ws_ = (float*)hip_.mem(ws_total * sizeof(float));
        l2_ws_ = (float*)hip_.mem(l2norm_bwd_ws_floats(B * 64 * 64, 512) * sizeof(float));
        size_t pws = 0;
        for (auto& op : ops_)
            if (op.kind == OP_POOL) {
                const Tensor& in = tensors_[op.in];
                const Tensor& out = tensors_[op.out];
                PoolDesc d{B, in.H, in.W, in.C, out.H, out.W, op.k, op.stride, op.pad_h, op.pad_w};
                pws = std::max(pws, maxpool_bwd_ws_bytes(d));
            }
        pool_ws_ = hip_.mem(pws);
        for (auto& op : ops_)
            if (op.kind == OP_POOL) {
                const Tensor& in = tensors_[op.in];
                const Tensor& out = tensors_[op.out];
                PoolDesc d{B, in.H, in.W, in.C, out.H, out.W, op.k, op.stride, op.pad_h, op.pad_w};
                if (maxpool_rec_applicable(d) && in.consumers == 1) op.pool_rec = hip_.mem(maxpool_rec_bytes(d));
            }
    }
    result_ = (float*)hip_.mem((size_t)B * A * nv * sizeof(float));
    x_stage_ = (float*)hip_.mem((size_t)B * preset_->image_h * preset_->image_w * 3 * sizeof(float));
    y_stage_ = (float*)hip_.mem((size_t)B * A * nv * sizeof(float));
    loss_ws_ = hip_.mem(loss_work_bytes(B, A));
    loss_work_carve(lw_, loss_ws_, B, A);
    HIP_OK(hipMemset(loss_ws_, 0, loss_work_bytes(B, A)));
    void* dp = nullptr;
    losses_host_ = static_cast<float*>(hip_.pinned(LOSS_RING * 4 * sizeof(float), &dp));
    for (int i = 0; i < LOSS_RING * 4; ++i) losses_host_[i] = 0.f;
    losses_dev_ = static_cast<float*>(dp);
    lw_.losses = losses_dev_;
    for (int i = 0; i < LOSS_RING; ++i) ev_loss_[i] = hip_.event();
    anchors_dev_ = (double*)hip_.mem((size_t)A * 4 * sizeof(double));
    anchors_abs_dev_ = (int*)hip_.mem((size_t)A * 4 * sizeof(int));
    anchors_device(*preset_, anchors_dev_, anchors_abs_dev_, nullptr);
    HIP_OK(hipDeviceSynchronize());
}

static inline double urand(unsigned long long& s) {
    unsigned long long z = (s += 0x9E3779B97F4A7C15ull);
    z = (z ^ (z >> 30)) * 0xBF58476D1CE4E5B9ull;
    z = (z ^ (z >> 27)) * 0x94D049BB133111EBull;
    z ^= z >> 31;
    return (double)(z >> 11) * (1.0 / 9007199254740992.0);
}

void Net::init_weights(unsigned long long seed) {
    std::vector<float> h(nparams_, 0.f);
    unsigned long long s = seed * 0x2545F4914F6CDD1Dull + 1;
    for (const Variable& v : vars_) {
        if (v.ndim == 4) {
            const double fan_in = (double)v.shape[0] * v.shape[1] * v.shape[2];
            const double fan_out = (double)v.shape[0] * v.shape[1] * v.shape[3];
            const double lim = std::sqrt(6.0 / (fan_in + fan_out));
            for (size_t r = 0; r < v.rows; ++r)
                for (size_t c = 0; c < v.width; ++c) h[v.off + r * v.pitch + c] = (float)((urand(s) * 2.0 - 1.0) * lim);
        } else if (v.name == "l2_norm_conv4_3/scale") {
            for (size_t c = 0; c < v.width; ++c) h[v.off + c] = 20.f;
        }
    }
    HIP_OK(hipMemcpy(params_, h.data(), nparams_ * sizeof(float), hipMemcpyHostToDevice));
}

Net::Net(const char* preset, int num_classes, int max_batch, int device, bool training, unsigned long long seed,
         float* ext_params, float* ext_grads, float* ext_momentum, int dtype, int graph)
    : preset_(&get_preset(preset)), C_(num_classes), Bmax_(max_batch), device_(device), training_(training), bf16_(dtype >= 1 && dtype <= 4),
      fc_(graph == 1), quant_(dtype == 2 ? Quant::fp8 : dtype == 3 ? Quant::mxfp8 : dtype == 4 ? Quant::mxfp6 : Quant::none), hip_(device) {
    SSD_REQUIRE(dtype >= 0 && dtype <= 4, "dtype must be 0 (fp32), 1 (bf16), 2 (fp8), 3 (mxfp8) or 4 (mxfp6), got %d", dtype);
    SSD_REQUIRE(!(quant_ != Quant::none && training), "%s is inference only: create the handle with training = 0",
                quant_ == Quant::mxfp6 ? "SSD_DTYPE_MXFP6" : quant_ == Quant::mxfp8 ? "SSD_DTYPE_MXFP8" : "SSD_DTYPE_FP8");
    SSD_REQUIRE(graph == 0 || graph == 1, "graph must be 0 (a-trous) or 1 (fc), got %d", graph);
    require_num_classes(num_classes);
    SSD_REQUIRE(max_batch >= 1, "max_batch must be >= 1");
    HIP_OK(hipSetDevice(device));
    params_ = ext_params; grads_ = ext_grads; mom_ = ext_momentum;
    build_graph();
    alloc();
    init_weights(seed);
    const char* ov = getenv("SSD_OVERLAP_WGRAD");
    overlap_ = !(ov && ov[0] == '0');
    hstream_ = hip_.stream();
    ev_h_ = hip_.event();
    ev_cast_ = hip_.event();

    ev2_h_ = hip_.event();
    ev_l2_ = hip_.event();
    ev_join_ = hip_.event();
    ev_m2s_ = hip_.event();
    for (int i = 0; i < MAX_MAPS; ++i) ev2_fmap_[i] = hip_.event();
    for (int i = 0; i < MAX_MAPS; ++i) ev_fmap_[i] = hip_.event();
    if (training_) {
        wstream_ = hip_.stream();
        ev_dy_ = hip_.event();
        ev_w_ = hip_.event();
    }
    s2_ = training_ ? wstream_ : hip_.stream();
    if (quant_ != Quant::none) plan_fp8();
    plan_pool_fusion();
    plan_tail_chain();
    plan_winograd();
    if (training_)
        for (const Op& op : ops_)
            if (op.in != input_t_ && !tensors_[op.in].gev)
                tensors_[op.in].gev = hip_.event();
    bw_.begin(this);
}

Net::~Net() {
    if (g_prof == &prof_) g_prof = nullptr;
}

static char* at(const Tensor& t, int b0, bool grad = false) {
    return static_cast<char*>(grad ? t.grad : t.data) + (size_t)b0 * t.per_image() * ((grad ? t.grad_f32 : t.data_f32) ? 4 : 2);
}

static void quantize_q(Quant q, const Tensor& t, const void* src, int nb, QView dst, hipStream_t s) {
    switch (q) {
    case Quant::mxfp6: quantize_mxfp6(src, false, (size_t)nb * t.H * t.W, t.C, dst.codes, dst.scales, s); break;
    case Quant::mxfp8: quantize_mxfp8(src, false, (size_t)nb * t.H * t.W, t.C, dst.codes, dst.scales, s); break;
    case Quant::fp8: quantize_fp8(src, false, (size_t)nb * t.per_image(), dst.scale, dst.codes, s); break;
    case Quant::none: fail("quantize: the handle has no quantised format");
    }
}

static void quantize_filters_q(Quant q, const FilterQuantPlan& plan, const float* w, unsigned char* w8, float* sw8, unsigned char* wsc6, hipStream_t s) {
    if (q == Quant::mxfp6) quantize_filters_mxfp6(plan, w, w8, wsc6, s);
    else quantize_filters_fp8(plan, w, w8, sw8, s);
}

static void conv_fwd_q(Quant q, const ConvDesc& d, QView x, const unsigned char* w, const float* sw, const unsigned char* wsc, const float* bias,
                       void* y, QView y8, bool wants16, bool relu, hipStream_t s) {
    const int mx_mode = y8.codes ? (wants16 ? FP8_OUT_BF16_MX : FP8_OUT_MX) : FP8_OUT_BF16;
    switch (q) {
    case Quant::mxfp6:
        conv_fwd_mxfp6(d, x.codes, x.scales, w, wsc, bias, y, y8.codes, y8.scales, mx_mode, relu, s);
        break;
    case Quant::mxfp8:
        (conv_bigk(d) ? conv_bigk_fwd_mxfp8 : conv_fwd_mxfp8)(d, x.codes, x.scales, w, sw, bias, y, y8.codes, y8.scales, mx_mode, relu, s);
        break;
    case Quant::fp8:
        (conv_bigk(d) ? conv_bigk_fwd_fp8 : conv_fwd_fp8)(d, x.codes, w, x.scale, sw, bias, y, y8.codes,
                                                          y8.codes ? (wants16 ? FP8_OUT_BF16_E4M3 : FP8_OUT_E4M3) : FP8_OUT_BF16, y8.scale, relu, s);
        break;
    case Quant::none: fail("convolution: the handle has no quantised format");
    }
}

static void maxpool_fwd_q(Quant q, const PoolDesc& d, QView x, QView y, hipStream_t s) {
    switch (q) {
    case Quant::mxfp6: maxpool_fwd_mxfp6(d, x.codes, x.scales, y.codes, y.scales, s); break;
    case Quant::mxfp8: maxpool_fwd_mxfp8(d, x.codes, x.scales, y.codes, y.scales, s); break;
    case Quant::fp8: maxpool_fwd_fp8(d, x.codes, y.codes, s); break;
    case Quant::none: fail("max-pool: the handle has no quantised format");
    }
}

struct Net::LossSlotGuard {
    long long& seq;
    bool armed = false;
    bool done = false;
    explicit LossSlotGuard(long long& s) : seq(s) {}
    void failed() { if (armed && !done) { --seq; armed = false; } }
    ~LossSlotGuard() { if (armed && !done) --seq; }
// ... 218 lines not shown
}

void Net::forward_pool(FwdPass& p, int li, int op_index) {
    const Op& op = ops_[op_index];
    const Tensor& in = tensors_[op.in];
    const Tensor& out = tensors_[op.out];
    const Lane& ln = p.lane[li];
    if (op.fused_fwd) return;
    PoolDesc d{ln.nb, in.H, in.W, in.C, out.H, out.W, op.k, op.stride, op.pad_h, op.pad_w};
    if (op.pool_rec && p.train_mode) {
        void* rec = static_cast<char*>(op.pool_rec) + (size_t)ln.b0 * out.H * out.W * (in.C / 4) * sizeof(unsigned short);
        if (bf16_) maxpool_fwd_rec(d, reinterpret_cast<const bf16_t*>(at(in, ln.b0)), reinterpret_cast<bf16_t*>(at(out, ln.b0)), rec, ln.s);
        else maxpool_fwd_rec(d, reinterpret_cast<const float*>(at(in, ln.b0)), reinterpret_cast<float*>(at(out, ln.b0)), rec, ln.s);
    } else if (p.train_mode && pool_ws_ && maxpool_arg_applicable(d)) {
        void* arg = static_cast<char*>(pool_ws_) + (size_t)ln.b0 * out.H * out.W * (in.C / 4) * sizeof(unsigned);
        if (bf16_) maxpool_fwd_arg(d, reinterpret_cast<const bf16_t*>(at(in, ln.b0)), reinterpret_cast<bf16_t*>(at(out, ln.b0)), arg, ln.s);
        else maxpool_fwd_arg(d, reinterpret_cast<const float*>(at(in, ln.b0)), reinterpret_cast<float*>(at(out, ln.b0)), arg, ln.s);
        pool_arg_op_ = op_index;
    } else if (p.run8 && op.fp8) {
        maxpool_fwd_q(quant_, d, q_at(in, ln.b0), q_at(out, ln.b0), ln.s);
        if (out.wants16) maxpool_fwd(d, reinterpret_cast<const bf16_t*>(at(in, ln.b0)), reinterpret_cast<bf16_t*>(at(out, ln.b0)), ln.s);
    } else if (bf16_) {
        maxpool_fwd(d, reinterpret_cast<const bf16_t*>(at(in, ln.b0)), reinterpret_cast<bf16_t*>(at(out, ln.b0)), ln.s);
        if (p.run8 && out.data8)
            quantize_q(quant_, out, at(out, ln.b0), ln.nb, q_at(out, ln.b0), ln.s);
    } else maxpool_fwd(d, reinterpret_cast<const float*>(at(in, ln.b0)), reinterpret_cast<float*>(at(out, ln.b0)), ln.s);
}

void Net::forward_l2norm(FwdPass& p, int li, int op_index) {
    const Op& op = ops_[op_index];
    const Tensor& in = tensors_[op.in];
    const Tensor& out = tensors_[op.out];
    const Lane& ln = p.lane[li];
    if (bf16_) l2norm_fwd(ln.nb * in.H * in.W, in.C, reinterpret_cast<const bf16_t*>(at(in, ln.b0)), params_ + scale_off_,
                          reinterpret_cast<bf16_t*>(at(out, ln.b0)), ln.s);
    else l2norm_fwd(ln.nb * in.H * in.W, in.C, reinterpret_cast<const float*>(at(in, ln.b0)), params_ + scale_off_,
                    reinterpret_cast<float*>(at(out, ln.b0)), ln.s);
}

void Net::forward_loss(FwdPass& p, const float* y, LossSlotGuard& guard) {
    const int b = p.b;
    const bool train_mode = p.train_mode;
    prof_.layer = "loss";
    const int A = preset_->num_anchors, nv = C_ + 5;
    if (train_mode) { bw_loss_kind_ = loss_kind_; bw_gamma_ = focal_gamma_; bw_alpha_ = focal_alpha_; bw_loc_ = loc_; }
    const bool focal = train_mode && bw_loss_kind_ == 1;
    try {
    if (p.heads_full) {
        HIP_OK(hipEventRecord(ev_h_, hstream_));
        HIP_OK(hipStreamWaitEvent(stream_, ev_h_, 0));
        HIP_OK(hipEventRecord(ev_join_, s2_));
        HIP_OK(hipStreamWaitEvent(stream_, ev_join_, 0));
        if (focal) multibox_focal_loss(heads_, b, 0, b, result_, y, lw_, wd_, loss_bnorm_, bw_gamma_, bw_alpha_, stream_, bw_loc_);
        else if (train_mode) multibox_loss(heads_, b, 0, b, result_, y, lw_, wd_, loss_bnorm_, stream_, bw_loc_);
        else heads_result(heads_, b, result_, stream_);
    }
    for (int li = 0; li < p.nl && !p.heads_full; ++li) {
        Lane& ln = p.lane[li];
        if (ln.heads_on_side) {
            HIP_OK(hipEventRecord(ln.ev_h, ln.h));
            HIP_OK(hipStreamWaitEvent(ln.s, ln.ev_h, 0));
        }
        HeadLayout hl = heads_;
        for (int i = 0; i < hl.nmaps; ++i) hl.buf[i] = heads_.buf[i] + (size_t)ln.b0 * hl.hw[i] * hl.ld[i];
        float* res = result_ + (size_t)ln.b0 * A * nv;
        if (train_mode) {
            if (li == 1) HIP_OK(hipStreamWaitEvent(ln.s, ev_l2_, 0));
            if (focal) multibox_focal_loss(hl, ln.nb, ln.b0, b, res, y + (size_t)ln.b0 * A * nv, lw_, wd_, loss_bnorm_, bw_gamma_, bw_alpha_, ln.s, bw_loc_);
            else multibox_loss(hl, ln.nb, ln.b0, b, res, y + (size_t)ln.b0 * A * nv, lw_, wd_, loss_bnorm_, ln.s, bw_loc_);
        } else {
            heads_result(hl, ln.nb, res, ln.s);
        }
    }
    } catch (...) {
        if (train_mode && lw_.ticket) {
            (void)hipDeviceSynchronize();
            (void)hipMemset(lw_.ticket, 0, sizeof(unsigned));
        }
        guard.failed();
        throw;
    }
}

void Net::launch_wgrad(int op_index, int b, hipStream_t ws) {
    const Op& op = ops_[op_index];
    const Tensor& in = tensors_[op.in];
    const Tensor& out = tensors_[op.out];
    const ConvDesc d = conv_desc(op, b);
    float* slab = wgrad_ws_ + op.ws_off;
    prof_.layer = op.name.c_str();
    if (op.wino_w && op.wino_v_step == fwd_serial_) {
        const size_t tpi = (size_t)wino_tiles(d) / d.B;
        wino_bwd_transform(d, out.gf(), nullptr, wino_ya_, ws);
        wino_wgrad(d, op.wino_V, (size_t)b * tpi * d.Ci, wino_ya_, grads_ + op.w_off, grads_ + op.b_off, params_ + op.w_off, wd_,
                   wino_slab_, ws);
    } else if (!bf16_) {
        conv_wgrad(d, in.f(), out.gf(), grads_ + op.w_off, grads_ + op.b_off, params_ + op.w_off, wd_, slab, ws);
    } else if (in.data_f32) {
        if (first_layer_kernel(d))
            conv_first_wgrad_bf16(d, in.f(), out.gh(), grads_ + op.w_off, grads_ + op.b_off, params_ + op.w_off, wd_, slab, ws);
        else
            conv_wgrad_smallc_bf16dy(d, in.f(), out.gh(), grads_ + op.w_off, grads_ + op.b_off, params_ + op.w_off, wd_, slab, ws);
    } else {
        conv_wgrad_bf16(d, in.h(), out.gh(), grads_ + op.w_off, grads_ + op.b_off, params_ + op.w_off, wd_, slab, ws);
    }
}

void Net::launch_dgrad(const Op& op, const ConvDesc& d, const Op* up, Tensor& dst, bool mask, int cls, hipStream_t ds) {
    const Tensor& in = tensors_[op.in];
    const Tensor& out = tensors_[op.out];
    if (op.wino_d && cls == 0) {
        wino_bwd_transform(d, out.gf(), wino_yt_, nullptr, ds);
        wino_dgrad(d, wino_yt_, op.wino_Uf, up ? dst.gf() : in.gf(), mask ? in.f() : nullptr, !up && in.done > 0, wino_xw_,
                   up ? up->pool_rec : nullptr, dst.H, dst.W, ds,
                   op.wino_bits && op.wino_bits_step == fwd_serial_ ? op.wino_bits : nullptr);
    } else if (!bf16_) {
        if (up) conv_dgrad_unpool(d, out.gf(), params_ + op.w_off, dst.gf(), up->pool_rec, dst.H, dst.W, ds);
        else conv_dgrad(d, out.gf(), params_ + op.w_off, in.gf(), mask ? in.f() : nullptr, in.done > 0, ds);
    } else {
        if (up) conv_dgrad_unpool_bf16(d, out.gh(), wq_io_ + op.w_off, dst.gh(), up->pool_rec, dst.H, dst.W, ds);
        else conv_dgrad_bf16(d, out.gh(), wq_io_ + op.w_off, in.gh(), mask ? in.h() : nullptr, in.done > 0, ds);
    }
}

void Net::backward_begin(int b, const float* y) {
    SSD_REQUIRE(training_, "handle was created with training = 0");
    g_prof = &prof_;
    prof_.layer = "loss";
    const bool side = hstream_ && overlap_;
    for (Tensor& t : tensors_) { t.done = 0; t.gstream = 0; t.gseq = 0; t.gev_set = false; }
    bw_issued_[0] = bw_issued_[1] = 0;
    bw_seen_[0][0] = bw_seen_[0][1] = bw_seen_[1][0] = bw_seen_[1][1] = 0;
    if (wino_flip_pending_) {
        HIP_OK(hipStreamWaitEvent(stream_, ev_wino_flip_, 0));
        wino_flip_pending_ = false;
    }
    if (bw_loss_kind_ == 1) multibox_focal_loss_grad(heads_, b, 0, result_, y, lw_, bw_gamma_, bw_alpha_, stream_, bw_loc_);
    else multibox_loss_grad(heads_, b, 0, result_, y, lw_, stream_, bw_loc_);
    for (int t : head_t_) bw_wrote(0, tensors_[t]);
    if (side) bw_sync(1, 0);
    bw_.begin(this);
    bw_first_on_main_ = false;
    bw_first_fused_ = false;
    bw_b_ = b;
}

bool Net::backward_step(size_t min_floats, size_t* off, size_t* count, bool sync_main) {
    const int b = bw_b_;
    bool side_used = false;
    for (int op_index; (op_index = bw_.next(min_floats)) >= 0;) {
        const Op& op = ops_[op_index];
        Tensor& in = tensors_[op.in];
        const Tensor& out = tensors_[op.out];
        const bool need_dx = op.in != input_t_;
        const bool last = in.done + 1 == in.consumers;
        prof_.layer = op.name.c_str();
        const int cls = bw_class(op, op_index);
        hipStream_t ds = cls == 1 ? hstream_ : stream_;
        if (chain_bwd_ && in_chain_[op_index] && !op_ablated(op.name, op.kind, op.head, op.k)) {
            if (!bw_.chain_done) {
                launch_tail_backward(b, &side_used);
                prof_.layer = op.name.c_str();
            }
            if (op_index != chain_first_) continue;
        }
        if (op_ablated(op.name, op.kind, op.head, op.k)) {
            bw_.retire(op_index);
            in.done++;
            continue;
        }
        switch (op.kind) {
        case OP_CONV: {
            const ConvDesc d = conv_desc(op, b);
            const bool side = wstream_ && overlap_;
            const bool on_main = side && !need_dx;
            hipStream_t ws = (side && !on_main) ? wstream_ : stream_;
            if (side && !on_main) {
                if (out.gev && out.gev_set) {
                    HIP_OK(hipStreamWaitEvent(wstream_, out.gev, 0));
                } else {
                    const bool from_side = out.gstream == 1 || (cls == 1 && bw_seen_[1][0] >= out.gseq);
                    HIP_OK(hipEventRecord(ev_dy_, from_side ? hstream_ : stream_));
                    HIP_OK(hipStreamWaitEvent(wstream_, ev_dy_, 0));
                }
                side_used = true;
            } else {
                bw_need(0, out);
                if (on_main) bw_first_on_main_ = true;
            }
            if (!(bw_first_fused_ && !need_dx))
                launch_wgrad(op_index, b, ws);
            if (need_dx) {
                bw_need(cls, out);
                const Op* up = op.unpool >= 0 ? &ops_[op.unpool] : nullptr;
                Tensor& dst = up ? tensors_[up->in] : in;
                if (!up && in.done > 0) bw_need(cls, in);
                const bool mask = !up && last && in.relu_out;
                int first = -1;
                if (fuse_first_wgrad_ && !up && mask && in.done == 0)
                    for (int j = 0; j < (int)ops_.size(); ++j)
                        if (ops_[j].kind == OP_CONV && ops_[j].out == op.in && ops_[j].in == input_t_) first = j;
                if (first >= 0 && cls == 0 && conv_dgrad_first_wgrad_bf16_applicable(d, conv_desc(ops_[first], b))) {
                    const Op& f = ops_[first];
                    prof_.layer = "conv1_2+conv1_1";
                    conv_dgrad_first_wgrad_bf16(d, out.gh(), wq_io_ + op.w_off, in.h(), conv_desc(f, b), tensors_[input_t_].f(),
                                                grads_ + f.w_off, grads_ + f.b_off, params_ + f.w_off, wd_, wgrad_ws_ + f.ws_off, ds);
                    bw_first_fused_ = true;
                    fused_first_out_ = op.in;
                    bw_wrote(cls, in);
                    bw_.retire(op_index);
                    break;
                }
                g_stop_event = dst.gev;
                struct Disarm { ~Disarm() { g_stop_event = nullptr; } } disarm;
                launch_dgrad(op, d, up, dst, mask, cls, ds);
                const bool carried = dst.gev && g_stop_event == nullptr;
                bw_wrote(cls, dst, carried);
            }
            bw_.retire(op_index);
            break;
        }
        case OP_POOL: {
            if (op.fused_bwd) break;
            bw_need(0, out);
            if (in.done > 0) bw_need(0, in);
            PoolDesc d{b, in.H, in.W, in.C, out.H, out.W, op.k, op.stride, op.pad_h, op.pad_w};
            void* pws = maxpool_bwd_ws_bytes(d) ? pool_ws_ : nullptr;
            if (op.pool_rec && in.done == 0 && last) {
                if (bf16_) maxpool_bwd_rec(d, op.pool_rec, out.gh(), in.gh(), in.relu_out, stream_);
                else maxpool_bwd_rec(d, op.pool_rec, out.gf(), in.gf(), in.relu_out, stream_);
            } else if (pool_arg_op_ == op_index && pws && maxpool_arg_applicable(d)) {
                if (bf16_) maxpool_bwd_arg(d, in.h(), pws, out.gh(), in.gh(), in.done > 0, last && in.relu_out, stream_);
                else maxpool_bwd_arg(d, in.f(), pws, out.gf(), in.gf(), in.done > 0, last && in.relu_out, stream_);
            } else if (bf16_)
                maxpool_bwd(d, in.h(), out.gh(), in.gh(), in.done > 0, last && in.relu_out, pws, stream_);
            else
                maxpool_bwd(d, in.f(), out.gf(), in.gf(), in.done > 0, last && in.relu_out, pws, stream_);
            bw_wrote(0, in);
            break;
        }
        case OP_L2NORM: {
            SSD_REQUIRE(in.done == 0 && !last, "l2norm backward must be the first of several consumers");
            bw_need(cls, out);
            if (bf16_)
                l2norm_bwd(b * in.H * in.W, in.C, in.h(), params_ + scale_off_, out.gh(), in.gh(), grads_ + scale_off_, l2_ws_, ds);
            else
                l2norm_bwd(b * in.H * in.W, in.C, in.f(), params_ + scale_off_, out.gf(), in.gf(), grads_ + scale_off_, l2_ws_, ds);
            bw_wrote(cls, in);
            break;
        }
        }
        in.done++;
    }
    const bool finished = bw_.finished();
    if (finished && bw_issued_[1] > bw_seen_[0][1]) bw_sync(0, 1);
    if (wstream_ && overlap_ && (side_used || finished) && (sync_main || finished)) {
        HIP_OK(hipEventRecord(ev_w_, wstream_));
        HIP_OK(hipStreamWaitEvent(stream_, ev_w_, 0));
    }
    if (wstream_ && !sync_main && (!overlap_ || (finished && bw_first_on_main_))) {
        HIP_OK(hipEventRecord(ev_dy_, stream_));
        HIP_OK(hipStreamWaitEvent(wstream_, ev_dy_, 0));
    }
    const std::pair<size_t, size_t> range = bw_.end_stage();
    *off = range.first;
    *count = range.second;
    return !finished;
}

std::vector<std::pair<size_t, size_t>> Net::backward_ranges(size_t min_floats) const {
    std::vector<std::pair<size_t, size_t>> out;
    BwProgress p;
    p.begin(this);
    while (!p.finished()) {
        for (int i; (i = p.next(min_floats)) >= 0;) p.retire(i);
        const std::pair<size_t, size_t> range = p.end_stage();
        if (range.second > 0) out.push_back(range);
    }
    return out;
}

void Net::set_wgrad_stream(hipStream_t s) {
    SSD_REQUIRE(training_, "handle was created with training = 0");
    hip_.free_stream(wstream_);
    wstream_ = s;
    s2_ = s;
}

void Net::backward(int b, const float* y) {
    backward_begin(b, y);
    size_t off, count;
    while (backward_step(nparams_, &off, &count, true)) {}
}

float Net::current_lr() const {
    for (size_t i = 0; i < lr_bounds_.size(); ++i)
        if (global_step <= lr_bounds_[i]) return lr_values_[i];
    return lr_values_[lr_bounds_.size()];
// ... 279 lines not shown
```

### ssd_tensorflow_amd/csrc/winograd.hip

```cpp
#include "conv.h"
#include "conv_detail.h"
#include "bf16.h"
#include <algorithm>
#include <cmath>

namespace ssd {

#define LDS_PTR(p) ((__attribute__((address_space(3))) void*)(p))
constexpr unsigned WOOB = 0xFFFFFFF0u;

__device__ __forceinline__ void bt6(f32x4& d0, f32x4& d1, f32x4& d2, f32x4& d3, f32x4& d4, f32x4& d5) {
    const f32x4 t0 = 1.265625f * d0 - 2.8125f * d2 + d4;
    const f32x4 e = d4 - 2.25f * d2, f = 1.6875f * d1 - 0.75f * d3;
    const f32x4 g = d4 - 0.5625f * d2, h = 0.84375f * d1 - 1.5f * d3;
    const f32x4 t5 = 1.265625f * d1 - 2.8125f * d3 + d5;
    d0 = t0; d1 = e - f; d2 = e + f; d3 = g - h; d4 = g + h; d5 = t5;
}
__device__ __forceinline__ void a6(const f32x4 e0, const f32x4 e1, const f32x4 e2, const f32x4 e3, f32x4* u) {
    const f32x4 p = e0 + 0.5625f * e2, q = 0.75f * e1 + 0.421875f * e3;
    const f32x4 r = e0 + 2.25f * e2, t = 1.5f * e1 + 3.375f * e3;
    u[0] = e0;
    u[1] = p + q;
    u[2] = p - q;
    u[3] = r + t;
// ... 178 lines not shown
        }
    } else if constexpr (MODE == 2) {
#pragma unroll
        for (int wr = 0; wr < 2; ++wr) {
            const int ph = 2 * i + wr;
            if (ph >= p.PH) continue;
            const bool okh = 4 * i + 2 * wr + 1 < p.H;
#pragma unroll
            for (int wc = 0; wc < 2; ++wc) {
                const int pw = 2 * j + wc;
                if (pw >= p.PW) continue;
                const bool okw = 4 * j + 2 * wc + 1 < p.W;
                const bool ok[4] = {true, okw, okh, okw && okh};
                V mm = o[2 * wr][2 * wc];
                unsigned rec = 0;
#pragma unroll
                for (int e = 0; e < 4; ++e) {
                    unsigned a = 0;
                    float best = mm[e];
#pragma unroll
                    for (int cq = 1; cq < 4; ++cq) {
                        const float v = o[2 * wr + (cq >> 1)][2 * wc + (cq & 1)][e];
                        if (ok[cq] && v > best) { best = v; a = cq; }
                    }
                    mm[e] = best;
                    rec |= (a | (best > 0.f ? 4u : 0u)) << (3 * e);
                }
                const size_t pix = (size_t)(b * p.PH + ph) * p.PW + pw;
                *reinterpret_cast<V*>(p.y + pix * p.N + ch) = mm;
                if (p.pool_rec) p.pool_rec[pix * c4n + q] = (unsigned short)rec;
            }
        }
    } else {
#pragma unroll
        for (int r = 0; r < 4; ++r) {
            const int h = 4 * i + r;
            if (h >= p.H) continue;
#pragma unroll
            for (int s = 0; s < 4; ++s) {
                const int w = 4 * j + s;
                if (w >= p.W) continue;
                const unsigned rec = p.unpool_rec[((size_t)(b * p.H + h) * p.W + w) * c4n + q];
#pragma unroll
                for (int cq = 0; cq < 4; ++cq) {
                    const int uh = 2 * h + (cq >> 1), uw = 2 * w + (cq & 1);
                    if (uh >= p.UH || uw >= p.UW) continue;
                    V v;
#pragma unroll
                    for (int e = 0; e < 4; ++e) {
                        const unsigned re = (rec >> (3 * e)) & 7u;
                        v[e] = ((re & 3u) == (unsigned)cq && (re & 4u)) ? o[r][s][e] : 0.f;
                    }
                    *reinterpret_cast<V*>(p.y + ((size_t)(b * p.UH + uh) * p.UW + uw) * p.N + ch) = v;
                }
            }
        }
    }
}

template <int MODE>
__global__ __launch_bounds__(256) void wino_out_kernel(WinoOutArgs p) {
    const int c4n = p.N >> 2;
    const int idx = blockIdx.x * 256 + threadIdx.x;
    const int q = idx % c4n, t = idx / c4n;
    if (t >= p.T) return;
    const float* src = p.M + (size_t)t * p.N + q * 4;
    f32x4 o[4][4];
    wino_out_transform([&](int r, int s) { return *reinterpret_cast<const f32x4*>(src + (size_t)(r * 6 + s) * p.m_ps); }, o);
    if constexpr (MODE == 0 || MODE == 2)
        wino_out_bias_relu(o, p.bias ? *reinterpret_cast<const f32x4*>(p.bias + q * 4) : f32x4{0.f, 0.f, 0.f, 0.f}, p.relu);
    wino_out_store<MODE>(p, t, q, o);
}

__device__ __forceinline__ void g6(const float g0, const float g1, const float g2, float* u) {
    u[0] = (64.f / 81.f) * g0;
    const float a = (-128.f / 243.f) * g0 - (8.f / 27.f) * g2, b = (32.f / 81.f) * g1;
    u[1] = a - b;
    u[2] = a + b;
    const float c = (32.f / 243.f) * g0 + (8.f / 27.f) * g2, d = (16.f / 81.f) * g1;
    u[3] = c + d;
    u[4] = c - d;
    u[5] = g2;
}
template <bool FLIP>
__global__ __launch_bounds__(256) void wino_filter_kernel(WinoFilterPlan plan) {
    int li = 0;
    for (int k = 1; k < plan.n; ++k)
        if ((int)blockIdx.x >= plan.it[k].blk0) li = k;
    const float* __restrict__ w = plan.it[li].w;
    float* __restrict__ U = FLIP ? plan.it[li].Uf : plan.it[li].U;
    if (!U) return;
    const int Ci = plan.it[li].Ci, Co = plan.it[li].Co;
    const int idx = ((int)blockIdx.x - plan.it[li].blk0) * 256 + threadIdx.x;
    if (idx >= Ci * Co) return;
    const int ci = FLIP ? idx % Ci : idx / Co, co = FLIP ? idx / Ci : idx % Co;
    float g[3][3];
#pragma unroll
    for (int a = 0; a < 3; ++a)
#pragma unroll
        for (int b = 0; b < 3; ++b) g[a][b] = w[((size_t)((FLIP ? 2 - a : a) * 3 + (FLIP ? 2 - b : b)) * Ci + ci) * Co + co];
    float c[6][3];
#pragma unroll
    for (int b = 0; b < 3; ++b) {
        float u[6];
        g6(g[0][b], g[1][b], g[2][b], u);
#pragma unroll
        for (int k = 0; k < 6; ++k) c[k][b] = u[k];
    }
    const size_t ps = FLIP ? (size_t)plan.it[li].Cop * Ci : (size_t)Ci * Co;
    const size_t e = FLIP ? (size_t)co * Ci + ci : (size_t)ci * Co + co;
#pragma unroll
    for (int k = 0; k < 6; ++k) {
        float u[6];
        g6(c[k][0], c[k][1], c[k][2], u);
#pragma unroll
        for (int l = 0; l < 6; ++l) U[(size_t)(k * 6 + l) * ps + e] = u[l];
    }
}

struct WinoGemmArgs {
    const float* A;
    const float* Bm;
    float* C;
    int M, N, K;
    size_t a_ps, b_ps, c_ps;
    int MT, NT;
};

template <int WM, int WN, int TM, int TN>
__global__ __launch_bounds__(256) void wino_gemm_nn_kernel(WinoGemmArgs p) {
    constexpr int BM = 32 * TM * WM, BN = 32 * TN * WN, BK = 32;
    constexpr int A_N = BM / 32;
    constexpr int B_CPR = BN / 4, B_RPP = 256 / B_CPR, B_N = BK / B_RPP;
    constexpr int A_BYTES = BM * 128, STAGE = (BM + BN) * 128;
    static_assert(WM * WN == 4, "4 waves per workgroup");
    static_assert(BK % B_RPP == 0, "filter tile vs staging pass");
    extern __shared__ __attribute__((aligned(16))) float smem[];
    unsigned char* const lds = reinterpret_cast<unsigned char*>(smem);
    const int tid = threadIdx.x;
    const int wave = __builtin_amdgcn_readfirstlane(tid >> 6), lane = tid & 63;
    int wg = xcd_remap(blockIdx.x, gridDim.x);
    const int nt = wg % p.NT;
    wg /= p.NT;
    const int mt = wg % p.MT, pos = wg / p.MT;
    const int m0 = mt * BM, n0 = nt * BN;

    const __amdgpu_buffer_rsrc_t a_rs = __builtin_amdgcn_make_buffer_rsrc(const_cast<float*>(p.A + (size_t)pos * p.a_ps), 0,
                                                                           (unsigned)((size_t)p.M * p.K * 4u), 0x00020000);
    const __amdgpu_buffer_rsrc_t b_rs = __builtin_amdgcn_make_buffer_rsrc(const_cast<float*>(p.Bm + (size_t)pos * p.b_ps), 0,
                                                                           (unsigned)((size_t)p.K * p.N * 4u), 0x00020000);
    const int a_c4 = ((tid & 7) ^ ((tid >> 4) & 7)) * 4;
    unsigned a_off[A_N], b_off[B_N];
#pragma unroll
    for (int i = 0; i < A_N; ++i) {
        const int m = m0 + (tid >> 3) + 32 * i;
        a_off[i] = m < p.M ? (unsigned)(m * p.K + a_c4) * 4u : WOOB;
    }
#pragma unroll
    for (int i = 0; i < B_N; ++i) {
        const int kr = tid / B_CPR + B_RPP * i, col = (tid % B_CPR) * 4;
        b_off[i] = n0 + col < p.N ? (unsigned)(kr * p.N + n0 + col) * 4u : WOOB;
    }
    const int nk = p.K / BK;
    auto issue = [&](int k, int stage) {
        unsigned char* As = lds + stage * STAGE + wave * 1024;
        unsigned char* Bs = lds + stage * STAGE + A_BYTES + wave * 1024;
        const int a_so = k * BK * 4, b_so = k * BK * p.N * 4;
#pragma unroll
        for (int i = 0; i < A_N; ++i) __builtin_amdgcn_raw_ptr_buffer_load_lds(a_rs, LDS_PTR(As + i * 4096), 16, (int)a_off[i], a_so, 0, 0);
#pragma unroll
        for (int i = 0; i < B_N; ++i) __builtin_amdgcn_raw_ptr_buffer_load_lds(b_rs, LDS_PTR(Bs + i * 4096), 16, (int)b_off[i], b_so, 0, 0);
    };

    f32x16 acc[TM][TN];
#pragma unroll
    for (int a = 0; a < TM; ++a)
#pragma unroll
        for (int b = 0; b < TN; ++b)
#pragma unroll
            for (int r = 0; r < 16; ++r) acc[a][b][r] = 0.f;
    const int wm = wave / WN, wn = wave - wm * WN;
    const int li = lane & 31, lh = lane >> 5;
    const int q0 = (lh ^ ((li >> 1) & 7)) * 16;
    const int a_row = (wm * 32 * TM + li) * 128 + q0;
    const int b_col = A_BYTES + (wn * 32 * TN + li) * 4;
    auto compute = [&](int stage) {
        const unsigned char* S = lds + stage * STAGE;
#pragma unroll
        for (int g = 0; g < BK / 8; ++g) {
            f32x4 a[TM], b[TN];
#pragma unroll
            for (int mi = 0; mi < TM; ++mi) a[mi] = *reinterpret_cast<const f32x4*>(S + ((a_row + mi * 4096) ^ (g * 32)));
            const int kb = g * 8 + lh * 4;
#pragma unroll
            for (int ni = 0; ni < TN; ++ni)
#pragma unroll
                for (int t = 0; t < 4; ++t) b[ni][t] = *reinterpret_cast<const float*>(S + b_col + ((kb + t) * BN + ni * 32) * 4);
#pragma unroll
            for (int t = 0; t < 4; ++t)
// ... 329 lines not shown
__global__ __launch_bounds__(36 * WR_E) void wino_wgrad_reduce36_kernel(const float* __restrict__ ws, int nsplit, int Ci, int Co,
                                                                        float* __restrict__ dw, float* __restrict__ db,
                                                                        const float* __restrict__ w, float wd) {
    __shared__ f32x4 sm[36][WR_E];
    __shared__ f32x4 cm[18][WR_E];
    const int c4n = Co >> 2, tid = threadIdx.x;
    const size_t cc = (size_t)Ci * Co, ucount = 36 * cc, stride = ucount + 16 * (size_t)Co;
    const int bias_blocks = (c4n + 31) / 32;
    if ((int)blockIdx.x < bias_blocks) {
        const int q = blockIdx.x * 32 + (tid & 31), slot = tid >> 5;
        if (!db) return;
        if (slot < 16 && q < c4n) {
            f32x4 t = {0.f, 0.f, 0.f, 0.f};
            for (int k = 0; k < nsplit; ++k) t += *reinterpret_cast<const f32x4*>(ws + (size_t)k * stride + ucount + (size_t)slot * Co + q * 4);
            (&sm[0][0])[slot * 32 + (tid & 31)] = t;
        }
        __syncthreads();
        if (slot == 0 && q < c4n) {
            f32x4 s = {0.f, 0.f, 0.f, 0.f};
            for (int sl = 0; sl < 16; ++sl) {
                const f32x4 t = (&sm[0][0])[sl * 32 + tid];
                s += (bias_axis_weight(sl >> 2) * bias_axis_weight(sl & 3)) * t;
            }
            *reinterpret_cast<f32x4*>(db + q * 4) = s;
        }
        return;
    }
    const int el = tid % WR_E, p = tid / WR_E;
    const int idx = (blockIdx.x - bias_blocks) * WR_E + el;
    const bool valid = idx < Ci * c4n;
    const size_t e = (size_t)idx * 4;
    f32x4 wv[3];
    const bool last = p < 3 && valid;
    if (last && wd != 0.f) {
#pragma unroll
        for (int b = 0; b < 3; ++b) wv[b] = *reinterpret_cast<const f32x4*>(w + (size_t)(p * 3 + b) * cc + e);
    }
    f32x4 s = {0.f, 0.f, 0.f, 0.f};
    if (valid) {
        for (int sp0 = 0; sp0 < nsplit; sp0 += 4) {
            f32x4 v[4];
#pragma unroll
            for (int u = 0; u < 4; ++u) v[u] = *reinterpret_cast<const f32x4*>(ws + (size_t)min(sp0 + u, nsplit - 1) * stride + (size_t)p * cc + e);
#pragma unroll
            for (int u = 0; u < 4; ++u)
                if (sp0 + u < nsplit) s += v[u];
        }
    }
    sm[p][el] = s;
    __syncthreads();
    if (p < 6) {
        f32x4 g[3];
        gt3(sm[p][el], sm[6 + p][el], sm[12 + p][el], sm[18 + p][el], sm[24 + p][el], sm[30 + p][el], g);
#pragma unroll
        for (int a = 0; a < 3; ++a) cm[a * 6 + p][el] = g[a];
    }
    __syncthreads();
    if (last) {
        f32x4 g[3];
        gt3(cm[p * 6][el], cm[p * 6 + 1][el], cm[p * 6 + 2][el], cm[p * 6 + 3][el], cm[p * 6 + 4][el], cm[p * 6 + 5][el], g);
#pragma unroll
        for (int b = 0; b < 3; ++b) {
            f32x4 v = g[b];
            if (wd != 0.f) v += wd * wv[b];
            *reinterpret_cast<f32x4*>(dw + (size_t)(p * 3 + b) * cc + e) = v;
        }
    }
}

static int tiles_1d(int n, int dil) { return dil * cdiv(cdiv(n, dil), 4); }
bool wino_applicable(const ConvDesc& d) {
    return d.KH == 3 && d.KW == 3 && d.stride == 1 && d.dil >= 1 && d.pad_h == d.dil && d.pad_w == d.dil && d.Ho == d.Hi && d.Wo == d.Wi &&
           d.Ci % 32 == 0 && d.Co % 4 == 0 && wino_tiles(d) >= 1 &&
           (long long)wino_tiles(d) * std::max(d.Ci, wino_kpad(d.Co)) < (1LL << 30) - 4 &&
           (long long)d.B * d.Hi * d.Wi * std::max(d.Ci, d.Co) < (1LL << 30) - 4;
}
int wino_kpad(int c) { return (c + 31) / 32 * 32; }
int wino_tiles(const ConvDesc& d) { return d.B * tiles_1d(d.Ho, d.dil) * tiles_1d(d.Wo, d.dil); }

static void require(const ConvDesc& d) { SSD_REQUIRE(wino_applicable(d), "winograd: 3x3 / stride 1 / SAME layers (any dilation), Ci in multiples of 32, Co of 4"); }

void WinoFilterPlan::add(const float* w, float* U, float* Uf, int Ci, int Co) {
    SSD_REQUIRE(n < MAX, "winograd: more than %d layers in one filter plan", MAX);
    it[n] = Item{w, U, Uf, Ci, Co, wino_kpad(Co), blocks};
    blocks += cdiv((long long)Ci * Co, 256);
    elems += (double)Ci * Co;
    ++n;
}
void wino_filter_plan(const WinoFilterPlan& plan, bool forward, bool flipped, hipStream_t s) {
    if (plan.n == 0) return;
    const double by = 4.0 * plan.elems * (9 + 36);
    if (forward) {
        ProfScope prof("wino_filter", 0, by, s);
        hipLaunchKernelGGL(wino_filter_kernel<false>, dim3(plan.blocks), dim3(256), 0, s, plan);
    }
    if (flipped) {
        ProfScope prof("wino_filter_flip", 0, by, s);
        hipLaunchKernelGGL(wino_filter_kernel<true>, dim3(plan.blocks), dim3(256), 0, s, plan);
    }
    HIP_OK(hipGetLastError());
}
void wino_filter(const ConvDesc& d, const float* w, float* U, float* Uflip, hipStream_t s) {
    require(d);
    WinoFilterPlan plan;
    plan.add(w, U, Uflip, d.Ci, d.Co);
    wino_filter_plan(plan, U != nullptr, Uflip != nullptr, s);
}

enum { GEOM_IN = 0, GEOM_REDUCE = 1 };
static bool ref_geometry(bool asked, int part) {
    static const int on = env_int("SSD_WINO_GEOMETRY", 1);
    return asked || on == 0 || (on == 2 && part != GEOM_IN) || (on == 3 && part != GEOM_REDUCE);
}

static void launch_in(const float* x, float* V, float* Va, int B, int H, int W, int C, int Cp, int D, size_t v_ps, size_t va_ps, hipStream_t s,
                      unsigned long long* bits, bool raster) {
    const int th = tiles_1d(H, D), tw = tiles_1d(W, D), T = B * th * tw;
    const unsigned xb = (unsigned)((size_t)B * H * W * C * 4u);
    const int grid = cdiv((long long)T * (Cp / 4), 256);
    const double by = 4.0 * ((double)B * H * W * C + 36.0 * T * Cp * ((V ? 1 : 0) + (Va ? 1 : 0)));
    if (V && Va) {
        launch_in(x, V, nullptr, B, H, W, C, Cp, D, v_ps, 0, s, bits, raster);
        launch_in(x, nullptr, Va, B, H, W, C, Cp, D, 0, va_ps, s, nullptr, raster);
        return;
    } else if (V) {
        ProfScope prof("wino_in", 0, by, s);
        hipLaunchKernelGGL((wino_in_kernel<true, false>), dim3(grid), dim3(256), 0, s, x, V, Va, H, W, C, Cp, th, tw, T, xb, v_ps, va_ps, D, bits, raster);
    } else {
        ProfScope prof("wino_in_wgrad", 0, by, s);
        hipLaunchKernelGGL((wino_in_kernel<false, true>), dim3(grid), dim3(256), 0, s, x, V, Va, H, W, C, Cp, th, tw, T, xb, v_ps, va_ps, D, bits, raster);
    }
    HIP_OK(hipGetLastError());
}

template <int WM, int WN, int TM, int TN>
static void launch_nn(WinoGemmArgs& a, const char* label, hipStream_t s) {
    constexpr int BM = 32 * TM * WM, BN = 32 * TN * WN;
    constexpr size_t lds = 2 * (size_t)(BM + BN) * 128;
    auto kern = wino_gemm_nn_kernel<WM, WN, TM, TN>;
    static bool once = (set_lds(kern, lds), true);
    (void)once;
    a.MT = cdiv(a.M, BM);
    a.NT = cdiv(a.N, BN);
    ProfScope prof(label, 2.0 * 36 * a.M * (double)a.N * a.K, 4.0 * 36 * ((double)a.M * a.K + (double)a.K * a.N + (double)a.M * a.N), s);
    hipLaunchKernelGGL(kern, dim3(36 * a.MT * a.NT), dim3(256), lds, s, a);
    HIP_OK(hipGetLastError());
}

static void gemm_nn(const float* A, size_t a_ps, const float* Bm, float* C, size_t c_ps, int M, int N, int K, hipStream_t s) {
    WinoGemmArgs a{};
    a.A = A; a.Bm = Bm; a.C = C; a.M = M; a.N = N; a.K = K;
    a.a_ps = a_ps; a.b_ps = (size_t)K * N; a.c_ps = c_ps;
    static const int forced = env_int("SSD_WINO_TILE", -1);
    int cfg = 0;
    if (forced >= 0) cfg = forced;
    else if (cdiv(N, 64) * 64 < cdiv(N, 128) * 128) cfg = 1;
    else if ((double)cdiv(M, 128) * 128 > 1.06 * M && (double)cdiv(M, 64) * 64 < (double)cdiv(M, 128) * 128) cfg = 2;
    switch (cfg) {
    case 0: launch_nn<2, 2, 2, 2>(a, "wino_gemm_128x128", s); break;
    case 1: launch_nn<4, 1, 1, 2>(a, "wino_gemm_128x64", s); break;
    case 2: launch_nn<2, 2, 1, 2>(a, "wino_gemm_64x128", s); break;
    default: launch_nn<2, 2, 1, 1>(a, "wino_gemm_64x64", s); break;
    }
}

template <int MODE>
static void launch_out(WinoOutArgs& a, const char* label, double bytes, hipStream_t s) {
    ProfScope prof(label, 0, bytes, s);
    SSD_LAUNCH_STOP(wino_out_kernel<MODE>, dim3(cdiv((long long)a.T * (a.N / 4), 256)), dim3(256), 0, s, a);
    HIP_OK(hipGetLastError());
}

static bool fuse_out(const ConvDesc& d, int N, int K, bool two_launch) {
    static const int on = env_int("SSD_WINO_FUSE_OUT", 1);
    return on && !two_launch && d.dil == 1 && (N == 64 || N == 128) && (K == 64 || K == 128) && !(N == 128 && K == 128);
}
template <int MODE>
static void launch_fused(const float* A, size_t a_ps, const float* Bm, int K, const WinoOutArgs& o, double out_bytes, hipStream_t s) {
    constexpr size_t lds = 4 * (size_t)(32 * 64 + 64 * 64) * 4;
    WinoFusedArgs a{};
    a.A = A; a.Bm = Bm; a.M = o.T; a.N = o.N; a.K = K; a.a_ps = a_ps; a.b_ps = (size_t)K * o.N; a.NT = o.N / 64; a.out = o;
    ProfScope prof("wino_gemm_out_32x64", 2.0 * 36 * a.M * (double)a.N * a.K, 4.0 * 36 * ((double)a.M * a.K + (double)a.K * a.N) + out_bytes, s);
    if (K == 64) {
        auto kern = wino_gemm_out_kernel<MODE, 1>;
        static bool once = (set_lds(kern, lds), true);
        (void)once;
        SSD_LAUNCH_STOP(kern, dim3(cdiv(a.M, 32) * a.NT), dim3(512), lds, s, a);
    } else {
        auto kern = wino_gemm_out_kernel<MODE, 2>;
        static bool once = (set_lds(kern, lds), true);
        (void)once;
        SSD_LAUNCH_STOP(kern, dim3(cdiv(a.M, 32) * a.NT), dim3(512), lds, s, a);
    }
    HIP_OK(hipGetLastError());
}

size_t wino_fwd_ws_floats(const ConvDesc& d) { return (size_t)36 * wino_tiles(d) * d.Co; }

void wino_fwd(const ConvDesc& d, const float* x, const float* U, const float* bias, float* y, bool relu, float* V, size_t v_ps,
              float* Mws, float* y_pool, void* pool_rec, hipStream_t s, void* relu_bits, bool two_launch, bool ref_geom) {
    require(d);
    const int T = wino_tiles(d);
    launch_in(x, V, nullptr, d.B, d.Hi, d.Wi, d.Ci, d.Ci, d.dil, v_ps, 0, s, static_cast<unsigned long long*>(relu_bits), ref_geometry(ref_geom, GEOM_IN));
    const bool fused = fuse_out(d, d.Co, d.Ci, two_launch);
    if (!fused) gemm_nn(V, v_ps, U, Mws, (size_t)T * d.Co, T, d.Co, d.Ci, s);
    WinoOutArgs a{};
    a.M = Mws; a.m_ps = (size_t)T * d.Co; a.bias = bias; a.relu = relu; a.H = d.Ho; a.W = d.Wo; a.N = d.Co;
    a.th = tiles_1d(d.Ho, d.dil); a.tw = tiles_1d(d.Wo, d.dil); a.T = T; a.D = d.dil;
    const double mb = 4.0 * 36 * T * d.Co;
    if (y_pool) {
        SSD_REQUIRE(d.dil == 1, "winograd: the fused pool is for undilated layers");
        a.y = y_pool; a.pool_rec = static_cast<unsigned short*>(pool_rec); a.PH = (d.Ho + 1) / 2; a.PW = (d.Wo + 1) / 2;
        const double ob = 4.0 * d.B * a.PH * a.PW * d.Co;
        if (fused) launch_fused<2>(V, v_ps, U, d.Ci, a, ob, s);
        else launch_out<2>(a, "wino_out_pool", mb + ob, s);
    } else {
        a.y = y;
        const double ob = 4.0 * d.B * d.Ho * d.Wo * d.Co;
        if (fused) launch_fused<0>(V, v_ps, U, d.Ci, a, ob, s);
        else launch_out<0>(a, "wino_out", mb + ob, s);
    }
}

size_t wino_dgrad_ws_floats(const ConvDesc& d) { return (size_t)36 * wino_tiles(d) * d.Ci; }

void wino_bwd_transform(const ConvDesc& d, const float* dy, float* Yt, float* Ya, hipStream_t s, bool ref_geom) {
    require(d);
    const size_t ps = (size_t)wino_tiles(d) * wino_kpad(d.Co);
    launch_in(dy, Yt, Ya, d.B, d.Ho, d.Wo, d.Co, wino_kpad(d.Co), d.dil, ps, ps, s, nullptr, ref_geometry(ref_geom, GEOM_IN));
}

void wino_dgrad(const ConvDesc& d, const float* Yt, const float* Uflip, float* dx, const float* mask, bool accumulate, float* Xws,
                const void* unpool_rec, int UH, int UW, hipStream_t s, const void* mask_bits, bool two_launch) {
    require(d);
    const int T = wino_tiles(d);
    const size_t yt_ps = (size_t)T * wino_kpad(d.Co);
    const bool fused = fuse_out(d, d.Ci, wino_kpad(d.Co), two_launch);
    if (!fused) gemm_nn(Yt, yt_ps, Uflip, Xws, (size_t)T * d.Ci, T, d.Ci, wino_kpad(d.Co), s);
    WinoOutArgs a{};
    a.M = Xws; a.m_ps = (size_t)T * d.Ci; a.y = dx; a.mask = mask; a.accum = accumulate; a.H = d.Hi; a.W = d.Wi; a.N = d.Ci;
    a.mask_bits = mask ? static_cast<const unsigned long long*>(mask_bits) : nullptr;
    a.th = tiles_1d(d.Hi, d.dil); a.tw = tiles_1d(d.Wi, d.dil); a.T = T; a.D = d.dil;
    const double mb = 4.0 * 36 * T * d.Ci;
    if (unpool_rec) {
        SSD_REQUIRE(d.dil == 1, "winograd: the un-pooling form is for undilated layers");
        a.unpool_rec = static_cast<const unsigned short*>(unpool_rec); a.UH = UH; a.UW = UW;
        const double ob = 4.0 * d.B * UH * UW * d.Ci;
        if (fused) launch_fused<3>(Yt, yt_ps, Uflip, wino_kpad(d.Co), a, ob, s);
        else launch_out<3>(a, "wino_out_unpool", mb + ob, s);
    } else {
        const double ob = 4.0 * d.B * d.Hi * d.Wi * d.Ci * (mask && !a.mask_bits ? 2 : 1);
        if (fused) launch_fused<1>(Yt, yt_ps, Uflip, wino_kpad(d.Co), a, ob, s);
        else launch_out<1>(a, "wino_out_dgrad", mb + ob, s);
    }
}

static void tn_tile(const ConvDesc& d, int* bk, int* bn) {
    *bk = d.Ci <= 64 ? 64 : 128;
    *bn = d.Co <= 64 ? 64 : 128;
}
static int tn_splits(const ConvDesc& d) {
    const int T = wino_tiles(d);
    int bk, bn;
    tn_tile(d, &bk, &bn);
    const int base = 36 * cdiv(d.Ci, bk) * cdiv(d.Co, bn);
    const double slots = 256.0 * std::min(8, (int)(160 * 1024 / (2 * 32 * (bk + bn) * 4)));
    const double it_us = 3.4 * (bk * bn) / (128.0 * 128.0) * slots / 512.0;
    int best = 1;
    double bc = 1e300;
    for (int ns = 1; ns <= 16; ++ns) {
        const int chunk = cdiv(cdiv(T, ns), 32) * 32;
        if (ns > 1 && chunk < 128) break;
        const double rounds = std::ceil((double)base * ns / slots);
        const double cost = rounds * (chunk / 32) * it_us + (ns > 1 ? 2.0 * ns * 36.0 * d.Ci * d.Co * 4.0 / 4.0e6 : 0.0);
        if (cost < bc) { bc = cost; best = ns; }
    }
    return best;
}
size_t wino_wgrad_ws_floats(const ConvDesc& d) { return (size_t)tn_splits(d) * ((size_t)36 * d.Ci * d.Co + 16 * (size_t)d.Co); }

template <int WM, int WN, int TM, int TN>
static void launch_tn(WinoTnArgs& a, const char* label, double flops, double bytes, hipStream_t s) {
    constexpr int BKT = 32 * TM * WM, BNT = 32 * TN * WN;
    constexpr size_t lds = 2 * (size_t)32 * (BKT + BNT) * 4;
    auto kern = wino_gemm_tn_kernel<WM, WN, TM, TN>;
    static bool once = (set_lds(kern, lds), true);
    (void)once;
    a.CT = cdiv(a.Ci, BKT); a.NT = cdiv(a.Co, BNT);
    ProfScope prof(label, flops, bytes, s);
    hipLaunchKernelGGL(kern, dim3(36 * a.CT * a.NT * a.nsplit), dim3(256), lds, s, a);
    HIP_OK(hipGetLastError());
}

void wino_wgrad(const ConvDesc& d, const float* V, size_t v_ps, const float* Ya, float* dw, float* dbias, const float* w,
                float weight_decay, float* ws, hipStream_t s, bool ref_geom) {
    require(d);
    const int T = wino_tiles(d);
    WinoTnArgs a{};
    a.X = V; a.Y = Ya; a.ws = ws; a.T = T; a.Ci = d.Ci; a.Co = d.Co; a.x_ps = v_ps; a.y_ps = (size_t)T * wino_kpad(d.Co);
    a.x_ld = d.Ci; a.y_ld = wino_kpad(d.Co);
    a.nsplit = tn_splits(d);
    a.tchunk = cdiv(cdiv(T, a.nsplit), 32) * 32;
    a.nsplit = cdiv(T, a.tchunk);
    SSD_REQUIRE((size_t)a.nsplit <= (size_t)tn_splits(d), "winograd: split plan");
    const double fl = 2.0 * 36 * T * (double)d.Ci * d.Co, by = 4.0 * 36 * ((double)T * (d.Ci + d.Co) + (double)a.nsplit * d.Ci * d.Co);
    int bk, bn;
    tn_tile(d, &bk, &bn);
    if (bk == 128 && bn == 128) launch_tn<2, 2, 2, 2>(a, "wino_gemm_tn_128x128", fl, by, s);
    else if (bk == 64 && bn == 128) launch_tn<2, 2, 1, 2>(a, "wino_gemm_tn_64x128", fl, by, s);
    else if (bk == 128 && bn == 64) launch_tn<4, 1, 1, 2>(a, "wino_gemm_tn_128x64", fl, by, s);
    else launch_tn<2, 2, 1, 1>(a, "wino_gemm_tn_64x64", fl, by, s);
    {
// ... 14 lines not shown
```

Baseline: 1439 images/s.

## Share one dual-output Winograd dy transform between dgrad and wgrad, LDS filter flip

For layers that need both dgrad and wgrad, the backward dy Winograd input transform now runs once on the main stream in a single kernel that writes both the dgrad layout and the wgrad layout. The wgrad on the side stream consumes the shared buffer. Two wgrad buffers are used alternately, with events guarding reuse, so consecutive layers do not serialize on one buffer. This replaces a second read and transform of dy on the side stream. In exchange the transform moves onto the critical main stream, and the extra buffer costs memory. The flipped filter transform also gets an LDS-tiled kernel so weight reads are coalesced.

```diff
diff --git a/include/ssdvgg_hip.h b/include/ssdvgg_hip.h
--- a/include/ssdvgg_hip.h
+++ b/include/ssdvgg_hip.h
@@ -337,6 +337,7 @@
 int ssd_detect_host(ssd_handle h, int which, const int** count, const float** conf, const int** cls, const int** idx,
                     const int** box, int* b, int* out_cap);
 int ssd_set_overlap(ssd_handle h, int on);
+int ssd_set_wino_dual(ssd_handle h, int mode);
 int ssd_profile_enable(ssd_handle h, int on);
 int ssd_profile_report(ssd_handle h, char* buf, size_t cap);
 int ssd_activation_shape(ssd_handle h, const char* name, int* height, int* width, int* channels);
@@ -505,6 +506,8 @@
 int ssd_op_conv2d_wino_wgrad(const float* x, const float* dy, float* dw, float* dbias, const float* w, float weight_decay, float* ws,
                              int flags, int b, int hi, int wi, int ci, int ho, int wo, int co, int kh, int kw, int stride, int dil,
                              int pad_h, int pad_w, void* stream);
+int ssd_op_wino_bwd_transform(const float* dy, float* Yt, float* Ya, int b, int h, int w, int co, int dil, int flags, void* stream);
+int ssd_op_wino_filter_flip_plan(const float* const* w, float* const* Uf, const int* ci, const int* co, int n, int flags, void* stream);
 int ssd_pool_fusion(ssd_handle h, int* out, int cap, int* count);
 int ssd_debug_set_ablate(const char* tokens);
 
diff --git a/ssd_tensorflow_amd/_lib.py b/ssd_tensorflow_amd/_lib.py
--- a/ssd_tensorflow_amd/_lib.py
+++ b/ssd_tensorflow_amd/_lib.py
@@ -177,6 +177,7 @@
     'ssd_detout_tiles_merge_dev': (i32, [i32, vp, i32, i32, i32, i32, i32, vp, vp, vp, vp, vp, vp, vp, sz, vp]),
     'ssd_detout_tiles': (i32, [cstr, i32, i32, vp, vp, i32, i32, f32, i32, i32, i32, i32, vp, vp, vp, vp, vp, vp]),
     'ssd_set_overlap': (i32, [handle, i32]),
+    'ssd_set_wino_dual': (i32, [handle, i32]),
     'ssd_profile_enable': (i32, [handle, i32]),
     'ssd_profile_report': (i32, [handle, C.c_char_p, sz]),
     'ssd_activation_shape': (i32, [handle, cstr, p_i32, p_i32, p_i32]),
@@ -190,6 +191,8 @@
     'ssd_op_conv2d_wino_fwd': (i32, [vp, vp, vp, vp, vp, vp, vp, vp, i32] + [i32] * 14 + [vp]),
     'ssd_op_conv2d_wino_dgrad': (i32, [vp, vp, vp, vp, vp, i32, vp, i32, i32, vp, i32] + [i32] * 13 + [vp]),
     'ssd_op_conv2d_wino_wgrad': (i32, [vp, vp, vp, vp, vp, f32, vp, i32] + [i32] * 13 + [vp]),
+    'ssd_op_wino_bwd_transform': (i32, [vp, vp, vp, i32, i32, i32, i32, i32, i32, vp]),
+    'ssd_op_wino_filter_flip_plan': (i32, [vp, vp, vp, vp, i32, i32, vp]),
     'ssd_op_cast_filter': (i32, [vp, vp, vp, i32, i32, i32, vp]),
     'ssd_op_conv2d_fwd_bf16': (i32, [vp, vp, vp, vp, i32] + [i32] * 14 + [vp]),
     'ssd_op_conv2d_dgrad_bf16': (i32, [vp, vp, vp, vp, i32] + [i32] * 13 + [vp]),
diff --git a/ssd_tensorflow_amd/csrc/api.hip b/ssd_tensorflow_amd/csrc/api.hip
--- a/ssd_tensorflow_amd/csrc/api.hip
+++ b/ssd_tensorflow_amd/csrc/api.hip
@@ -1389,6 +1389,12 @@
     API_END
 }
 
+int ssd_set_wino_dual(ssd_handle h, int on) {
+    API_BEGIN_NET(h)
+    n.set_wino_dual(on);
+    API_END
+}
+
 int ssd_profile_enable(ssd_handle h, int on) {
     API_BEGIN_NET(h)
     n.profiler().on = on != 0;
@@ -1688,6 +1694,21 @@
     }
     wino_bwd_transform(d, dy, nullptr, k.Ya, (hipStream_t)stream, (flags & 8) != 0);
     wino_wgrad(d, k.V, vps, k.Ya, dw, dbias, w, weight_decay, k.slabs, (hipStream_t)stream, (flags & 8) != 0);
+    API_END
+}
+int ssd_op_wino_bwd_transform(const float* dy, float* Yt, float* Ya, int b, int h, int w, int co, int dil, int flags, void* stream) {
+    API_BEGIN
+    const ConvDesc d = mk(b, h, w, 32, h, w, co, 3, 3, 1, dil, dil, dil);
+    SSD_REQUIRE(wino_applicable(d), "winograd: 3x3 / stride 1 / SAME layers (any dilation), Ci in multiples of 32, Co of 4");
+    SSD_REQUIRE(Yt && Ya, "ssd_op_wino_bwd_transform: both outputs are required");
+    wino_bwd_transform(d, dy, Yt, Ya, (hipStream_t)stream, (flags & 8) != 0, (flags & 16) != 0);
+    API_END
+}
+int ssd_op_wino_filter_flip_plan(const float* const* w, float* const* Uf, const int* ci, const int* co, int n, int flags, void* stream) {
+    API_BEGIN
+    WinoFilterPlan plan;
+    for (int i = 0; i < n; ++i) plan.add(w[i], nullptr, Uf[i], ci[i], co[i]);
+    wino_filter_plan(plan, false, true, (hipStream_t)stream, (flags & 1) != 0);
     API_END
 }
 size_t ssd_op_conv2d_wgrad_ws_floats(int b, int hi, int wi, int ci, int ho, int wo, int co, int kh, int kw, int stride,
diff --git a/ssd_tensorflow_amd/csrc/conv.h b/ssd_tensorflow_amd/csrc/conv.h
--- a/ssd_tensorflow_amd/csrc/conv.h
+++ b/ssd_tensorflow_amd/csrc/conv.h
@@ -44,17 +44,18 @@
         const float* w;
         float *U, *Uf;
         int Ci, Co, Cop, blk0;
+        int tblk0;
     } it[MAX];
-    int n = 0, blocks = 0;
+    int n = 0, blocks = 0, tblocks = 0;
     double elems = 0;
     void add(const float* w, float* U, float* Uf, int Ci, int Co);
 };
-void wino_filter_plan(const WinoFilterPlan& plan, bool forward, bool flipped, hipStream_t s);
+void wino_filter_plan(const WinoFilterPlan& plan, bool forward, bool flipped, hipStream_t s, bool flip_lanes_ci = false);
 size_t wino_fwd_ws_floats(const ConvDesc& d);
 void wino_fwd(const ConvDesc& d, const float* x, const float* U, const float* bias, float* y, bool relu, float* V, size_t v_ps,
               float* Mws, float* y_pool, void* pool_rec, hipStream_t s, void* relu_bits = nullptr, bool two_launch = false,
               bool ref_geom = false);
-void wino_bwd_transform(const ConvDesc& d, const float* dy, float* Yt, float* Ya, hipStream_t s, bool ref_geom = false);
+void wino_bwd_transform(const ConvDesc& d, const float* dy, float* Yt, float* Ya, hipStream_t s, bool ref_geom = false, bool two_launch = false);
 size_t wino_dgrad_ws_floats(const ConvDesc& d);
 void wino_dgrad(const ConvDesc& d, const float* Yt, const float* Uflip, float* dx, const float* mask, bool accumulate, float* Xws,
                 const void* unpool_rec, int UH, int UW, hipStream_t s, const void* mask_bits = nullptr, bool two_launch = false);
diff --git a/ssd_tensorflow_amd/csrc/net.h b/ssd_tensorflow_amd/csrc/net.h
--- a/ssd_tensorflow_amd/csrc/net.h
+++ b/ssd_tensorflow_amd/csrc/net.h
@@ -148,6 +148,7 @@
     long long global_step = 0;
     Profiler& profiler() { return prof_; }
     void set_overlap(bool on) { overlap_ = on; }
+    void set_wino_dual(int mode) { wino_dual_ = mode; }
 
 private:
     int add_tensor(const std::string& name, int H, int W, int C, bool relu_out);
@@ -206,8 +207,8 @@
     bool fuse_first_wgrad_ = false;
     bool bw_first_fused_ = false;
     int fused_first_out_ = -1;
-    void launch_wgrad(int op_index, int b, hipStream_t ws);
-    void launch_dgrad(const Op& op, const ConvDesc& d, const Op* up, Tensor& dst, bool mask, int cls, hipStream_t ds);
+    void launch_wgrad(int op_index, int b, hipStream_t ws, const float* ya = nullptr);
+    void launch_dgrad(const Op& op, const ConvDesc& d, const Op* up, Tensor& dst, bool mask, int cls, hipStream_t ds, bool yt_done = false);
     int chain_first_ = -1;
     std::vector<char> in_chain_;
     bf16_t* wq_tail_ = nullptr;
@@ -222,6 +223,12 @@
     bool wino_any_f_ = false, wino_any_d_ = false;
     float *wino_m_[3] = {nullptr, nullptr, nullptr}, *wino_vs_[3] = {nullptr, nullptr, nullptr}, *wino_yt_ = nullptr, *wino_xw_ = nullptr, *wino_ya_ = nullptr, *wino_slab_ = nullptr;
     hipEvent_t ev_wino_ = nullptr, ev_wino_first_ = nullptr, ev_wino_flip_ = nullptr;
+    float* wino_ya2_ = nullptr;
+    hipEvent_t ev_ya_free_[2] = {nullptr, nullptr};
+    bool ya_free_set_[2] = {false, false};
+    int ya_turn_ = 0;
+    int wino_dual_ = 1;
+    int wino_dual_max_c_ = 128;
     struct Lane {
         hipStream_t s, h;
         hipEvent_t* ev_fmap;
diff --git a/ssd_tensorflow_amd/csrc/net.hip b/ssd_tensorflow_amd/csrc/net.hip
--- a/ssd_tensorflow_amd/csrc/net.hip
+++ b/ssd_tensorflow_amd/csrc/net.hip
@@ -495,6 +495,7 @@
     const int mode = env_i("SSD_WINOGRAD", 15), min_cc = env_i("SSD_WINO_MIN_CC", 4096), head_min_hw = env_i("SSD_WINO_HEAD_MIN_HW", 16);
     if (!(mode & 7)) return;
     size_t m_max = 0, v_max = 0, yt_max = 0, xw_max = 0, slab_max = 0;
+    bool dual_any = false;
     for (Op& op : ops_) {
         if (op.kind != OP_CONV) continue;
         const ConvDesc d = conv_desc(op, Bmax_);
@@ -527,6 +528,7 @@
         if (op.wino_Uf) wino_plan_flip_.add(params_ + op.w_off, nullptr, op.wino_Uf, d.Ci, d.Co);
         wino_any_f_ |= op.wino_f;
         wino_any_d_ |= op.wino_d;
+        dual_any |= op.wino_d && op.wino_w;
     }
     if (wino_plan_.n + wino_plan_first_.n + wino_plan_flip_.n == 0) return;
     ev_wino_ = hip_.event();
@@ -539,6 +541,10 @@
         wino_xw_ = (float*)hip_.mem(xw_max * sizeof(float));
         wino_ya_ = (float*)hip_.mem(yt_max * sizeof(float));
         wino_slab_ = (float*)hip_.mem(slab_max * sizeof(float));
+        if (dual_any) {
+            wino_ya2_ = (float*)hip_.mem(yt_max * sizeof(float));
+            for (hipEvent_t& e : ev_ya_free_) e = hip_.event();
+        }
     }
 }
 
@@ -849,6 +855,8 @@
     init_weights(seed);
     const char* ov = getenv("SSD_OVERLAP_WGRAD");
     overlap_ = !(ov && ov[0] == '0');
+    wino_dual_ = env_i("SSD_WINO_DUAL", 1);
+    wino_dual_max_c_ = env_i("SSD_WINO_DUAL_MAX_C", wino_dual_max_c_);
     hstream_ = hip_.stream();
     ev_h_ = hip_.event();
     ev_cast_ = hip_.event();
@@ -1233,7 +1241,7 @@
     }
 }
 
-void Net::launch_wgrad(int op_index, int b, hipStream_t ws) {
+void Net::launch_wgrad(int op_index, int b, hipStream_t ws, const float* ya) {
     const Op& op = ops_[op_index];
     const Tensor& in = tensors_[op.in];
     const Tensor& out = tensors_[op.out];
@@ -1242,9 +1250,14 @@
     prof_.layer = op.name.c_str();
     if (op.wino_w && op.wino_v_step == fwd_serial_) {
         const size_t tpi = (size_t)wino_tiles(d) / d.B;
-        wino_bwd_transform(d, out.gf(), nullptr, wino_ya_, ws);
-        wino_wgrad(d, op.wino_V, (size_t)b * tpi * d.Ci, wino_ya_, grads_ + op.w_off, grads_ + op.b_off, params_ + op.w_off, wd_,
+        if (!ya) wino_bwd_transform(d, out.gf(), nullptr, wino_ya_, ws);
+        wino_wgrad(d, op.wino_V, (size_t)b * tpi * d.Ci, ya ? ya : wino_ya_, grads_ + op.w_off, grads_ + op.b_off, params_ + op.w_off, wd_,
                    wino_slab_, ws);
+        if (ws != stream_ && wino_ya2_) {
+            const int k = ya == wino_ya2_ ? 1 : 0;
+            HIP_OK(hipEventRecord(ev_ya_free_[k], ws));
+            ya_free_set_[k] = true;
+        }
     } else if (!bf16_) {
         conv_wgrad(d, in.f(), out.gf(), grads_ + op.w_off, grads_ + op.b_off, params_ + op.w_off, wd_, slab, ws);
     } else if (in.data_f32) {
@@ -1257,11 +1270,11 @@
     }
 }
 
-void Net::launch_dgrad(const Op& op, const ConvDesc& d, const Op* up, Tensor& dst, bool mask, int cls, hipStream_t ds) {
+void Net::launch_dgrad(const Op& op, const ConvDesc& d, const Op* up, Tensor& dst, bool mask, int cls, hipStream_t ds, bool yt_done) {
     const Tensor& in = tensors_[op.in];
     const Tensor& out = tensors_[op.out];
     if (op.wino_d && cls == 0) {
-        wino_bwd_transform(d, out.gf(), wino_yt_, nullptr, ds);
+        if (!yt_done) wino_bwd_transform(d, out.gf(), wino_yt_, nullptr, ds);
         wino_dgrad(d, wino_yt_, op.wino_Uf, up ? dst.gf() : in.gf(), mask ? in.f() : nullptr, !up && in.done > 0, wino_xw_,
                    up ? up->pool_rec : nullptr, dst.H, dst.W, ds,
                    op.wino_bits && op.wino_bits_step == fwd_serial_ ? op.wino_bits : nullptr);
@@ -1293,6 +1306,7 @@
     bw_.begin(this);
     bw_first_on_main_ = false;
     bw_first_fused_ = false;
+    ya_turn_ = 1;
     bw_b_ = b;
 }
 
@@ -1326,7 +1340,22 @@
             const bool side = wstream_ && overlap_;
             const bool on_main = side && !need_dx;
             hipStream_t ws = (side && !on_main) ? wstream_ : stream_;
-            if (side && !on_main) {
+            const bool dual = wino_dual_ && (wino_dual_ == 2 || std::max(d.Ci, d.Co) <= wino_dual_max_c_) && wino_ya2_ && need_dx && cls == 0 &&
+                              op.wino_d && op.wino_w && op.wino_v_step == fwd_serial_;
+            const float* ya = nullptr;
+            if (dual) {
+                bw_need(0, out);
+                float* buf = ya_turn_ ? wino_ya2_ : wino_ya_;
+                if (side && ya_free_set_[ya_turn_]) HIP_OK(hipStreamWaitEvent(stream_, ev_ya_free_[ya_turn_], 0));
+                wino_bwd_transform(d, out.gf(), wino_yt_, buf, stream_);
+                if (side) {
+                    HIP_OK(hipEventRecord(ev_dy_, stream_));
+                    HIP_OK(hipStreamWaitEvent(wstream_, ev_dy_, 0));
+                    side_used = true;
+                }
+                ya = buf;
+                ya_turn_ ^= 1;
+            } else if (side && !on_main) {
                 if (out.gev && out.gev_set) {
                     HIP_OK(hipStreamWaitEvent(wstream_, out.gev, 0));
                 } else {
@@ -1340,9 +1369,9 @@
                 if (on_main) bw_first_on_main_ = true;
             }
             if (!(bw_first_fused_ && !need_dx))
-                launch_wgrad(op_index, b, ws);
+                launch_wgrad(op_index, b, ws, ya);
             if (need_dx) {
-                bw_need(cls, out);
+                if (!dual) bw_need(cls, out);
                 const Op* up = op.unpool >= 0 ? &ops_[op.unpool] : nullptr;
                 Tensor& dst = up ? tensors_[up->in] : in;
                 if (!up && in.done > 0) bw_need(cls, in);
@@ -1364,7 +1393,7 @@
                 }
                 g_stop_event = dst.gev;
                 struct Disarm { ~Disarm() { g_stop_event = nullptr; } } disarm;
-                launch_dgrad(op, d, up, dst, mask, cls, ds);
+                launch_dgrad(op, d, up, dst, mask, cls, ds, dual);
                 const bool carried = dst.gev && g_stop_event == nullptr;
                 bw_wrote(cls, dst, carried);
             }
diff --git a/ssd_tensorflow_amd/csrc/winograd.hip b/ssd_tensorflow_amd/csrc/winograd.hip
--- a/ssd_tensorflow_amd/csrc/winograd.hip
+++ b/ssd_tensorflow_amd/csrc/winograd.hip
@@ -284,6 +284,23 @@
     u[4] = c - d;
     u[5] = g2;
 }
+__device__ __forceinline__ void wino_filter_store(const float (&g)[3][3], float* __restrict__ U, size_t ps, size_t e) {
+    float c[6][3];
+#pragma unroll
+    for (int b = 0; b < 3; ++b) {
+        float u[6];
+        g6(g[0][b], g[1][b], g[2][b], u);
+#pragma unroll
+        for (int k = 0; k < 6; ++k) c[k][b] = u[k];
+    }
+#pragma unroll
+    for (int k = 0; k < 6; ++k) {
+        float u[6];
+        g6(c[k][0], c[k][1], c[k][2], u);
+#pragma unroll
+        for (int l = 0; l < 6; ++l) U[(size_t)(k * 6 + l) * ps + e] = u[l];
+    }
+}
 template <bool FLIP>
 __global__ __launch_bounds__(256) void wino_filter_kernel(WinoFilterPlan plan) {
     int li = 0;
@@ -301,22 +318,42 @@
     for (int a = 0; a < 3; ++a)
 #pragma unroll
         for (int b = 0; b < 3; ++b) g[a][b] = w[((size_t)((FLIP ? 2 - a : a) * 3 + (FLIP ? 2 - b : b)) * Ci + ci) * Co + co];
-    float c[6][3];
-#pragma unroll
-    for (int b = 0; b < 3; ++b) {
-        float u[6];
-        g6(g[0][b], g[1][b], g[2][b], u);
-#pragma unroll
-        for (int k = 0; k < 6; ++k) c[k][b] = u[k];
-    }
     const size_t ps = FLIP ? (size_t)plan.it[li].Cop * Ci : (size_t)Ci * Co;
     const size_t e = FLIP ? (size_t)co * Ci + ci : (size_t)ci * Co + co;
-#pragma unroll
-    for (int k = 0; k < 6; ++k) {
-        float u[6];
-        g6(c[k][0], c[k][1], c[k][2], u);
-#pragma unroll
-        for (int l = 0; l < 6; ++l) U[(size_t)(k * 6 + l) * ps + e] = u[l];
+    wino_filter_store(g, U, ps, e);
+}
+
+__global__ __launch_bounds__(256) void wino_filter_flip_lds_kernel(WinoFilterPlan plan) {
+    __shared__ float sw[9][32][33];
+    int li = 0;
+    for (int k = 1; k < plan.n; ++k)
+        if ((int)blockIdx.x >= plan.it[k].tblk0) li = k;
+    const float* __restrict__ w = plan.it[li].w;
+    float* __restrict__ U = plan.it[li].Uf;
+    if (!U) return;
+    const int Ci = plan.it[li].Ci, Co = plan.it[li].Co;
+    const int tile = (int)blockIdx.x - plan.it[li].tblk0, nct = (Co + 31) / 32;
+    const int ci0 = (tile / nct) * 32, co0 = (tile % nct) * 32;
+    const int lane = threadIdx.x & 31, grp = threadIdx.x >> 5;
+#pragma unroll
+    for (int tap = 0; tap < 9; ++tap)
+#pragma unroll
+        for (int k = 0; k < 4; ++k) {
+            const int r = grp + 8 * k;
+            sw[tap][r][lane] = co0 + lane < Co ? w[((size_t)tap * Ci + ci0 + r) * Co + co0 + lane] : 0.f;
+        }
+    __syncthreads();
+    const size_t ps = (size_t)plan.it[li].Cop * Ci;
+#pragma unroll
+    for (int k = 0; k < 4; ++k) {
+        const int c = grp + 8 * k;
+        if (co0 + c >= Co) continue;
+        float g[3][3];
+#pragma unroll
+        for (int a = 0; a < 3; ++a)
+#pragma unroll
+            for (int b = 0; b < 3; ++b) g[a][b] = sw[(2 - a) * 3 + (2 - b)][lane][c];
+        wino_filter_store(g, U, ps, (size_t)(co0 + c) * Ci + ci0 + lane);
     }
 }
 
@@ -812,12 +849,15 @@
 
 void WinoFilterPlan::add(const float* w, float* U, float* Uf, int Ci, int Co) {
     SSD_REQUIRE(n < MAX, "winograd: more than %d layers in one filter plan", MAX);
-    it[n] = Item{w, U, Uf, Ci, Co, wino_kpad(Co), blocks};
+    SSD_REQUIRE(!Uf || Ci % 32 == 0, "winograd: the flipped filter transform takes Ci in multiples of 32 (got %d)", Ci);
+    it[n] = Item{w, U, Uf, Ci, Co, wino_kpad(Co), blocks, tblocks};
     blocks += cdiv((long long)Ci * Co, 256);
+    tblocks += (Ci / 32) * cdiv(Co, 32);
     elems += (double)Ci * Co;
     ++n;
 }
-void wino_filter_plan(const WinoFilterPlan& plan, bool forward, bool flipped, hipStream_t s) {
+void wino_filter_plan(const WinoFilterPlan& plan, bool forward, bool flipped, hipStream_t s, bool flip_lanes_ci) {
+    static const int flip_lds = env_int("SSD_WINO_FILTER_LDS", 1);
     if (plan.n == 0) return;
     const double by = 4.0 * plan.elems * (9 + 36);
     if (forward) {
@@ -826,7 +866,8 @@
     }
     if (flipped) {
         ProfScope prof("wino_filter_flip", 0, by, s);
-        hipLaunchKernelGGL(wino_filter_kernel<true>, dim3(plan.blocks), dim3(256), 0, s, plan);
+        if (flip_lanes_ci || !flip_lds) hipLaunchKernelGGL(wino_filter_kernel<true>, dim3(plan.blocks), dim3(256), 0, s, plan);
+        else hipLaunchKernelGGL(wino_filter_flip_lds_kernel, dim3(plan.tblocks), dim3(256), 0, s, plan);
     }
     HIP_OK(hipGetLastError());
 }
@@ -843,16 +884,24 @@
     return asked || on == 0 || (on == 2 && part != GEOM_IN) || (on == 3 && part != GEOM_REDUCE);
 }
 
+static bool dual_launch(bool two) {
+    static const int on = env_int("SSD_WINO_DUAL", 1);
+    return !two && on != 0;
+}
+
 static void launch_in(const float* x, float* V, float* Va, int B, int H, int W, int C, int Cp, int D, size_t v_ps, size_t va_ps, hipStream_t s,
-                      unsigned long long* bits, bool raster) {
+                      unsigned long long* bits, bool raster, bool two = false) {
     const int th = tiles_1d(H, D), tw = tiles_1d(W, D), T = B * th * tw;
     const unsigned xb = (unsigned)((size_t)B * H * W * C * 4u);
     const int grid = cdiv((long long)T * (Cp / 4), 256);
     const double by = 4.0 * ((double)B * H * W * C + 36.0 * T * Cp * ((V ? 1 : 0) + (Va ? 1 : 0)));
-    if (V && Va) {
+    if (V && Va && !dual_launch(two)) {
         launch_in(x, V, nullptr, B, H, W, C, Cp, D, v_ps, 0, s, bits, raster);
         launch_in(x, nullptr, Va, B, H, W, C, Cp, D, 0, va_ps, s, nullptr, raster);
         return;
+    } else if (V && Va) {
+        ProfScope prof("wino_in_dual", 0, by, s);
+        hipLaunchKernelGGL((wino_in_kernel<true, true>), dim3(grid), dim3(256), 0, s, x, V, Va, H, W, C, Cp, th, tw, T, xb, v_ps, va_ps, D, bits, raster);
     } else if (V) {
         ProfScope prof("wino_in", 0, by, s);
         hipLaunchKernelGGL((wino_in_kernel<true, false>), dim3(grid), dim3(256), 0, s, x, V, Va, H, W, C, Cp, th, tw, T, xb, v_ps, va_ps, D, bits, raster);
@@ -954,10 +1003,10 @@
 
 size_t wino_dgrad_ws_floats(const ConvDesc& d) { return (size_t)36 * wino_tiles(d) * d.Ci; }
 
-void wino_bwd_transform(const ConvDesc& d, const float* dy, float* Yt, float* Ya, hipStream_t s, bool ref_geom) {
+void wino_bwd_transform(const ConvDesc& d, const float* dy, float* Yt, float* Ya, hipStream_t s, bool ref_geom, bool two_launch) {
     require(d);
     const size_t ps = (size_t)wino_tiles(d) * wino_kpad(d.Co);
-    launch_in(dy, Yt, Ya, d.B, d.Ho, d.Wo, d.Co, wino_kpad(d.Co), d.dil, ps, ps, s, nullptr, ref_geometry(ref_geom, GEOM_IN));
+    launch_in(dy, Yt, Ya, d.B, d.Ho, d.Wo, d.Co, wino_kpad(d.Co), d.dil, ps, ps, s, nullptr, ref_geometry(ref_geom, GEOM_IN), two_launch);
 }
 
 void wino_dgrad(const ConvDesc& d, const float* Yt, const float* Uflip, float* dx, const float* mask, bool accumulate, float* Xws,
```

After: 1461 images/s (median of 6 runs). +1.6%, better.
